# Eurus-Holmes/VAG-NMT

Hardware: AMD Instinct MI355X
Metric: training sentence-pairs/sec (Multi30K en->de, B=64) (higher is better)
Workload: dtype f32; 1 GPU; configs[1]: multimodal en->de train step, B=64/GPU, Ts=Tt=40, E=256, H=512, S=512, I=2048, Vs=8507, V=9391, dropout 0.3/0.5/0.5, tied emb, teacher_force_ratio=1; global_batch=64, parallelism=dp1, hip_graph=True

## Files before the change

### vag-nmt_amd/csrc/api.hip

```cpp
#include "../../include/vag_nmt.h"
#include "api_shared.h"
#include <cstring>

static thread_local VagCallCtx g_base_ctx;
static thread_local VagCallCtx* g_active_ctx = nullptr;
VagCallCtx& vag_ctx() { return g_active_ctx ? *g_active_ctx : g_base_ctx; }
VagCallScope::VagCallScope(VagCallCtx& c) : ctx(c), prev(g_active_ctx) { g_active_ctx = &c; }
VagCallScope::~VagCallScope() {
    (void)vag_loss_defer_flush();
    if (ctx.leaf_on) vag_leaf_drop();
    g_active_ctx = prev;
}
static inline const float* as_f(const vag_half* p) { return reinterpret_cast<const float*>(p); }

VagOptions& vag_opt() {
    static VagOptions o;
    return o;
}

extern "C" {

int vag_version(void) { return 330; }

int vag_set_option(const char* name, int64_t value) {
// ... 45 lines not shown
                   float* d_x, int accumulate_dx, float* g_W, float* g_b, vag_stream_t stream) {
    hipStream_t s = S_(stream);
    VAG_CHECK_ARG(x && W && dy && M >= 0 && N > 0 && K > 0 && (!act || y));
    if (M == 0) return VAG_OK;
    if (act) VAG_TRY(vag_tanh_bwd_launch(y, dy, dy, M * N, nullptr, 0, 0.f, s));
    if (d_x) VAG_TRY(gemm_nn(M, K, N, dy, N, W, K, accumulate_dx ? 1.f : 0.f, d_x, K, s));
    if (g_W) VAG_TRY(gemm_tn_acc(N, K, M, dy, N, x, K, g_W, K, s));
    if (g_b) VAG_TRY(vag_colsum_launch(dy, M, N, N, g_b, s));
    return VAG_OK;
}

int vag_embed_fwd(const int64_t* idx, int64_t n, const float* W, int64_t E, float* out, vag_stream_t stream) {
    return vag_embed_gather_launch(idx, 1, 0, n, 1, W, E, out, nullptr, 0, 0.f, S_(stream));
}
int vag_embed_bwd(const int64_t* idx, int64_t n, const float* d_out, int64_t E, float* g_W, vag_stream_t stream) {
    return vag_embed_scatter_launch(idx, 1, 0, n, 1, d_out, E, g_W, nullptr, 0, 0.f, S_(stream));
}

struct DerivedW {
    float *prep, *wcatT, *whh1T, *encT;
    vag_half *wcat16, *wcatT16, *whh1_16, *whh1T16, *enc16, *encT16;
    int64_t total;
};
static int64_t cgru_prep_total(int64_t H);
static DerivedW derived_layout(float* p, int64_t H) {
    DerivedW w;
    const int64_t C = 2 * H, Q = C + 3 * H;
    WsCarver c(p);
    w.prep = c.take(cgru_prep_total(H)); w.wcatT = c.take(Q * H); w.whh1T = c.take(3 * H * H); w.encT = c.take(2 * 3 * H * H);
    w.wcat16 = c.take_as<vag_half>(Q * H); w.wcatT16 = c.take_as<vag_half>(Q * H);
    w.whh1_16 = c.take_as<vag_half>(3 * H * H); w.whh1T16 = c.take_as<vag_half>(3 * H * H);
    w.enc16 = c.take_as<vag_half>(2 * 3 * H * H); w.encT16 = c.take_as<vag_half>(2 * 3 * H * H);
    w.total = c.off;
    return w;
}

static float* handoff_planes(int64_t need) {
    const VagCallCtx& c = vag_ctx();
    return (need > 0 && c.handoff_planes && c.handoff_floats >= need) ? c.handoff_planes : nullptr;
}

struct BiGruWs {
    float *x, *xp, *hst, *gates, *dgh, *carry, *dx, *whhT, *gx;
    unsigned *sync, *sync_b;
    int64_t total;
};
static BiGruWs bigru_ws(float* ws, int64_t B, int64_t Ts, int64_t E, int64_t H) {
    BiGruWs w;
    WsCarver c(ws);
    w.x = c.take(Ts * B * E);
    w.xp = c.take(Ts * B * 6 * H);
    w.hst = c.take(2 * (Ts + 1) * B * H);
    w.gates = c.take(2 * Ts * 4 * B * H);
    w.dgh = c.take(2 * Ts * B * 3 * H);
    w.carry = c.take(4 * B * H);
    w.dx = c.take(Ts * B * E);
    w.whhT = c.take(2 * 3 * H * H);
    w.gx = c.take(3 * Ts * B * H);
    w.sync = c.take_as<unsigned>(vag_enc_persistent_sync_words(B, Ts));
    w.sync_b = c.take_as<unsigned>(vag_enc_persistent_sync_words(B, Ts));
    w.total = c.off;
    return w;
}
int64_t vag_bigru_ws_floats(int64_t B, int64_t Ts, int64_t E, int64_t H) { return bigru_ws(nullptr, B, Ts, E, H).total; }

int vag_bigru_seq_fwd(const int64_t* src, const int32_t* lengths, const float* emb, vag_gru_w fw, vag_gru_w bw, float p_emb,
                      float p_ctx, const uint64_t* rng, int64_t B, int64_t Ts, int64_t E, int64_t H, float* enc,
                      float* mask, float* ws, vag_stream_t stream) {
    hipStream_t s = S_(stream);
    VAG_CHECK_ARG(src && lengths && emb && enc && mask && ws && B > 0 && Ts > 0 && E > 0 && H > 0);
    VAG_CHECK_ARG(E % 4 == 0 && H % 4 == 0 && aligned16(ws) && aligned16(enc));
    VAG_CHECK_ARG(fw.w_ih && fw.w_hh && fw.b_ih && fw.b_hh && bw.w_ih && bw.w_hh && bw.b_ih && bw.b_hh);
    BiGruWs w = bigru_ws(ws, B, Ts, E, H);
    const int64_t R = Ts * B;
    VAG_TRY(vag_embed_gather_launch(src, 1, Ts, Ts, B, emb, E, w.x, rng, VAG_DROP_ENC_EMB, p_emb, s, mask));
    VagGemmGroup grp0;
    VAG_TRY(vag_gemm_launch(R, 3 * H, E, 1.f, w.x, E, 1, fw.w_ih, 1, E, 0.f, w.xp, 6 * H, fw.b_ih, 0, s));
    VAG_TRY(vag_gemm_launch(R, 3 * H, E, 1.f, w.x, E, 1, bw.w_ih, 1, E, 0.f, w.xp + 3 * H, 6 * H, bw.b_ih, 0, s));
    VAG_TRY(grp0.end(s));
    const int64_t BH = B * H;
    const bool s16 = vag_ctx().store16 && vag_ctx().derived;
    VAG_CHECK_ARG(!vag_ctx().store16 || (vag_ctx().derived && H % 8 == 0));
    if (!s16 && vag_opt().persistent && vag_enc_persistent_ok(B, Ts, H)) {
        return vag_enc_fwd_persistent_launch(w.xp, fw.w_hh, bw.w_hh, fw.b_hh, bw.b_hh, lengths, w.hst, w.gates, enc, w.sync, rng,
                                             p_ctx, B, Ts, H, s);
    }
    const vag_half* w16 = s16 ? derived_layout(const_cast<float*>(vag_ctx().derived), H).enc16 : nullptr;
    if (s16 && vag_opt().persistent && vag_enc_wide16_ok(B, Ts, H) && B >= 64) {
        return vag_enc_fwd_wide16_launch(w.xp, w16, w16 + 3 * H * H, fw.b_hh, bw.b_hh, lengths, w.hst, w.gates, enc,
                                         reinterpret_cast<vag_half*>(w.dgh), w.sync, rng, p_ctx, B, Ts, H, s);
    }
    {
        const VagJob zj[2] = {{nullptr, w.hst, B, H, H, H, 0}, {nullptr, w.hst + (Ts + 1) * BH, B, H, H, H, 0}};
        VAG_TRY(vag_jobs_launch(zj, 2, s));
    }
    GruStepArgs a = {};
    a.lda = H; a.ldw = H; a.ldother = 6 * H; a.ldh = H; a.ld2 = Ts * 2 * H;
    a.M = (int)B; a.K = (int)H; a.H = (int)H; a.lengths = lengths; a.comp_hidden = 1;
    for (int64_t k = 0; k < Ts; ++k) {
        for (int d = 0; d < 2; ++d) {
            const int64_t t = d == 0 ? k : Ts - 1 - k;
            const vag_gru_w& g = d == 0 ? fw : bw;
            float* hs = w.hst + d * (Ts + 1) * BH;
            GruSide& sd = a.s[d];
            sd.A = hs + k * BH; sd.W = s16 ? as_f(w16 + d * 3 * H * H) : g.w_hh; sd.bias = g.b_hh;
            sd.other = w.xp + t * B * 6 * H + d * 3 * H;
            sd.hprev = hs + k * BH; sd.hout = hs + (k + 1) * BH;
            sd.out2 = enc + t * 2 * H + d * H;
            sd.save = w.gates + (d * Ts + k) * 4 * BH;
            sd.t = (int)t;
        }
        VAG_TRY(vag_gru_step_launch(a, 2, s, s16));
    }
    VAG_TRY(vag_dropout_apply_launch(enc, B * Ts * 2 * H, 0, rng, VAG_DROP_ENC_CTX, p_ctx, s));
    return VAG_OK;
}

int vag_bigru_seq_bwd(const int64_t* src, const int32_t* lengths, vag_gru_w fw, vag_gru_w bw, float p_emb, float p_ctx,
                      const uint64_t* rng, int64_t B, int64_t Ts, int64_t E, int64_t H, float* d_enc, float* ws,
                      float* g_emb, vag_gru_g g_fw, vag_gru_g g_bw, vag_stream_t stream) {
    hipStream_t s = S_(stream);
    VAG_CHECK_ARG(src && lengths && d_enc && ws && g_emb && B > 0 && Ts > 0 && E % 4 == 0 && H % 4 == 0);
    BiGruWs w = bigru_ws(ws, B, Ts, E, H);
    const int64_t R = Ts * B, BH = B * H;
    float* d_xp = w.xp;
    const float* whhT = w.whhT;
    const bool s16 = vag_ctx().store16 && vag_ctx().derived;
    VAG_CHECK_ARG(!vag_ctx().store16 || (vag_ctx().derived && H % 8 == 0));
    if (s16) {
        whhT = as_f(derived_layout(const_cast<float*>(vag_ctx().derived), H).encT16);
    } else if (vag_ctx().derived) {
        whhT = derived_layout(const_cast<float*>(vag_ctx().derived), H).encT;
    } else {
        for (int d = 0; d < 2; ++d) {
            const vag_gru_w& g = d == 0 ? fw : bw;
            VAG_TRY(vag_transpose_launch(g.w_hh, 3 * H, H, w.whhT + d * 3 * H * H, s));
        }
    }
    const bool pers_on = vag_opt().persistent && vag_opt().persistent_enc_bwd;
    const bool wide16 = s16 && pers_on && vag_enc_wide16_ok(B, Ts, H) && B >= 64;
    const bool persist = wide16 || (!s16 && pers_on && (H == 512 || H == 256) && vag_enc_persistent_ok(B, Ts, H));
    if (wide16) {
        VAG_TRY(vag_enc_bwd_wide16_launch(reinterpret_cast<const vag_half*>(whhT), d_enc, w.gates, w.hst, lengths, rng, p_ctx, d_xp,
                                          w.dgh, reinterpret_cast<vag_half*>(w.gx), w.sync_b, B, Ts, H, s));
    } else if (persist) {
        VAG_TRY(vag_enc_bwd_persistent_launch(whhT, d_enc, w.gates, w.hst, lengths, rng, p_ctx, d_xp, w.dgh,
                                              handoff_planes(vag_enc_bwd_planes_floats(B, Ts, H)), w.sync_b, B, Ts, H, s));
    }
    GruBwdArgs a = {};
    a.ld_add = Ts * 2 * H; a.ldh = H; a.ldgi = 6 * H; a.ldgh = 3 * H;
    a.M = (int)B; a.H = (int)H; a.lengths = lengths; a.rng = rng; a.sid = VAG_DROP_ENC_CTX; a.p = p_ctx;
    int cur = 0;
    auto cell_of = [&](auto& sd, int d, int64_t k) {
        const int64_t t = d == 0 ? k : Ts - 1 - k;
        sd.dh_add = d_enc + t * 2 * H + d * H;
        sd.drop_idx0 = t * 2 * H + d * H;
        sd.save = w.gates + (d * Ts + k) * 4 * BH;
        sd.hprev = w.hst + (d * (Ts + 1) + k) * BH;
        sd.dgi = d_xp + t * B * 6 * H + d * 3 * H;
        sd.dgh = w.dgh + (d * Ts + k) * B * 3 * H;
        sd.t = (int)t;
    };
    for (int d = 0; d < 2; ++d) {
        GruBwdSide& sd = a.s[d];
        cell_of(sd, d, Ts - 1);
        sd.dh_carry = nullptr;
        sd.dh_prev = w.carry + (d * 2 + cur) * BH;
    }
// ... 381 lines not shown
}

struct CgruBwdScratch {
    float *wcatT, *wpT, *whh1T, *dgi2, *dqgh, *dalpha, *ds, *dgi1, *dgh1, *dh1d, *carry, *de, *dvp, *dwp, *dah, *dencwp, *pbuf;
    float *u_all, *du_all, *duk;
    int64_t total;
};
static CgruBwdScratch cgru_bwd_scratch(float* p, int64_t B, int64_t Ts, int64_t Tt, int64_t E, int64_t H) {
    CgruBwdScratch w;
    const int64_t C = 2 * H, Q = C + 3 * H, R = Tt * B;
    WsCarver c(p);
    w.wcatT = c.take(Q * H); w.wpT = c.take(3 * H * C); w.whh1T = c.take(3 * H * H);
    w.dgi2 = c.take(R * 3 * H); w.dqgh = c.take(R * Q);
    w.dalpha = c.take(B * Ts); w.ds = c.take(R * Ts);
    w.dgi1 = c.take(R * 3 * H); w.dgh1 = c.take(R * 3 * H);
    w.dh1d = c.take(B * H); w.carry = c.take(B * H); w.de = c.take(R * E); w.dvp = c.take(VAG_POST_CHUNKS(Ts) * B * C);
    w.dwp = c.take(3 * H * C);
    w.dah = c.take(R * Ts);
    w.dencwp = c.take(B * Ts * 3 * H);
    w.pbuf = c.take(B * H);
    w.u_all = c.take(R * H); w.du_all = c.take(R * H); w.duk = c.take(B * Ts * H);
    w.total = c.off;
    return w;
}
}
float* vag_cgru_bwd_scratch_de(float* scratch, int64_t B, int64_t Ts, int64_t Tt, int64_t E, int64_t H) {
    return cgru_bwd_scratch(scratch, B, Ts, Tt, E, H).de;
}
float* vag_cgru_bwd_scratch_du(float* scratch, int64_t B, int64_t Ts, int64_t Tt, int64_t E, int64_t H) {
    return cgru_bwd_scratch(scratch, B, Ts, Tt, E, H).du_all;
}
extern "C" {
int64_t vag_cgru_bwd_scratch_floats(int64_t B, int64_t Ts, int64_t Tt, int64_t E, int64_t H) {
    return cgru_bwd_scratch(nullptr, B, Ts, Tt, E, H).total;
}

int vag_cgru_attn_decode_seq_bwd_loop(const float* enc, const float* pe, const float* mask, const float* h0, const int64_t* tok,
                                 vag_dec_w w, int64_t B, int64_t Ts, int64_t Tt, int64_t E, int64_t H, int64_t V,
                                 const float* h2_all, const float* c_all, const float* e_all, float* d_h2_all,
                                 float* d_c_all, const float* d_e_all, float* ws, float* d_enc_out, int accumulate_enc,
                                 float* d_pe, float* d_h0, float* scratch, vag_stream_t stream) {
    hipStream_t s = S_(stream);
    VAG_CHECK_ARG(enc && pe && mask && h0 && tok && h2_all && c_all && e_all && d_h2_all && d_c_all && ws && d_enc_out &&
                  d_pe && d_h0 && scratch && dec_w_ok(w));
    VAG_CHECK_ARG(B > 0 && Ts > 0 && Tt > 0 && E % 4 == 0 && H % 4 == 0 && aligned16(ws) && aligned16(scratch));
    (void)V; (void)mask; (void)d_e_all;
    const int64_t C = 2 * H, Q = C + 3 * H, BH = B * H;
    CgruWs k = cgru_ws(ws, B, Ts, Tt, E, H);
    CgruPrep p = cgru_prep(k.prep, H);
    CgruBwdScratch z = cgru_bwd_scratch(scratch, B, Ts, Tt, E, H);
    const bool s16 = vag_ctx().store16;
    VAG_CHECK_ARG(!s16 || (vag_ctx().derived && H % 8 == 0));
    if (vag_ctx().derived) {
        DerivedW dw = derived_layout(const_cast<float*>(vag_ctx().derived), H);
        p = cgru_prep(dw.prep, H);
        z.wcatT = dw.wcatT; z.whh1T = dw.whh1T;
        if (s16) {
            z.wcatT = const_cast<float*>(as_f(dw.wcatT16)); z.whh1T = const_cast<float*>(as_f(dw.whh1T16));
        }
    } else {
        VAG_TRY(vag_transpose_launch(p.wcat, Q, H, z.wcatT, s));
        VAG_TRY(vag_transpose_launch(w.gru1.w_hh, 3 * H, H, z.whh1T, s));
    }
    const bool persist = !s16 && vag_opt().persistent && vag_opt().persistent_dec_bwd && vag_dec_bwd_persistent_ok(B, Ts, Tt, H);
    if (!persist) {
        GruBwdArgs a = {};
        a.ld_add = H; a.ldh = H; a.ldgi = 3 * H; a.ldgh = Q; a.M = (int)B; a.H = (int)H;
        const int64_t t = Tt - 1;
        GruBwdSide& sd = a.s[0];
        sd.dh_carry = nullptr; sd.dh_add = d_h2_all + t * BH; sd.drop_idx0 = 0;
        sd.save = k.g2 + t * 4 * BH; sd.hprev = k.h1 + t * BH;
        sd.dgi = z.dgi2 + t * B * 3 * H; sd.dgh = z.dqgh + t * B * Q + C; sd.dh_prev = z.dh1d; sd.t = 0;
        VAG_TRY(vag_gru_bwd_elem_launch(a, 1, s));
    }
    GruBwdStepArgs f = {};
    f.ld_add = H; f.ldh = H; f.M = (int)B; f.H = (int)H; f.lengths = nullptr; f.rng = nullptr; f.sid = 0; f.p = 0.f;
    if (C % 4 == 0 && aligned16(enc) && aligned16(d_c_all) && B < 65536)
        VAG_TRY(vag_skinny_batched_launch(B, Tt, Ts, C, d_c_all, B * C, C, enc, C, Ts * C, z.dah, B * Ts, Ts, s));
    else
        VAG_TRY(vag_attn_scores_ex_launch(1, enc, d_c_all, C, nullptr, nullptr, Tt * B, 1, B, Ts, C, nullptr, z.dah, s));
    if (persist) {
        VAG_TRY(vag_dec_bwd_persistent_launch(pe, k.encwp, w.attn_v, z.wcatT, z.whh1T, h0, h2_all, k.h1, k.g1, k.g2, k.qhp, k.alpha,
                                              d_h2_all, z.dah, z.dgi2, z.dqgh, z.ds, z.dgi1, z.dgh1, d_h0, k.dal,
                                              handoff_planes(vag_dec_bwd_planes_floats(B, Tt, H)), k.sync_b, B, Ts, Tt, H, s));
    }
    for (int64_t t = Tt - 1; t >= 0 && !persist; --t) {
        float* dgi2 = z.dgi2 + t * B * 3 * H;
        float* dqgh = z.dqgh + t * B * Q;
        const float* wside = s16 ? as_f(reinterpret_cast<const vag_half*>(z.wcatT) + C) : z.wcatT + C;
        VAG_TRY(vag_attn_dot_side_launch(1, k.encwp, dgi2, 3 * H, nullptr, nullptr, z.dah + t * B * Ts, B, Ts, 3 * H, z.dalpha,
                                         B, H, 3 * H, dqgh + C, Q, wside, Q, nullptr, z.dh1d, z.pbuf, H, s, s16));
        VAG_TRY(vag_attn_dq_launch(pe, k.qhp + t * B * Q, Q, w.attn_v, k.alpha + t * B * Ts, z.dalpha, z.ds + t * B * Ts, B,
                                   Ts, C, dqgh, Q, s, s16));
        f.lda = Q; f.ldw = Q; f.K = (int)C; f.ldgi = 3 * H; f.ldgh = 3 * H; f.has_cell = 1;
        GruBwdStepSide& sd = f.s[0];
        sd.A = dqgh; sd.WT = z.wcatT; sd.addend = z.pbuf; sd.dh_add = nullptr; sd.drop_idx0 = 0;
        sd.save = k.g1 + t * 4 * BH; sd.hprev = (t == 0) ? h0 : h2_all + (t - 1) * BH;
        sd.dgi = z.dgi1 + t * B * 3 * H; sd.dgh = z.dgh1 + t * B * 3 * H; sd.dh_direct = z.carry; sd.dh_out = nullptr; sd.t = 0;
        VAG_TRY(vag_gru_bwd_step_launch(f, 1, s, s16));
        f.lda = 3 * H; f.ldw = 3 * H; f.K = (int)(3 * H);
        sd.A = z.dgh1 + t * B * 3 * H; sd.WT = z.whh1T; sd.addend = z.carry;
        if (t > 0) {
            const int64_t t1 = t - 1;
            f.has_cell = 1; f.ldgi = 3 * H; f.ldgh = Q;
            sd.dh_add = d_h2_all + t1 * BH;
            sd.save = k.g2 + t1 * 4 * BH; sd.hprev = k.h1 + t1 * BH;
            sd.dgi = z.dgi2 + t1 * B * 3 * H; sd.dgh = z.dqgh + t1 * B * Q + C; sd.dh_direct = z.dh1d; sd.dh_out = nullptr;
        } else {
            f.has_cell = 0;
            sd.dh_add = nullptr; sd.save = nullptr; sd.hprev = nullptr; sd.dgi = nullptr; sd.dgh = nullptr;
            sd.dh_direct = nullptr; sd.dh_out = d_h0;
        }
        VAG_TRY(vag_gru_bwd_step_launch(f, 1, s, s16));
    }
    VAG_TRY(vag_attn_post_bwd_launch(pe, k.qhp, Q, w.attn_v, z.ds, k.alpha, d_c_all, B, Ts, Tt, C, d_pe, z.dvp, d_enc_out,
                                     accumulate_enc, s, s16));
    {
        VagGemmGroup now;
        VAG_TRY(gemm_nn(Tt * B, H, 3 * H, z.dgi2, 3 * H, w.gru2.w_ih, H, 0.f, z.du_all, H, s));
        VAG_TRY(now.end(s));
    }
    VAG_TRY(vag_attn_wsum_pair_launch(k.alpha, z.du_all, H, z.duk, k.uk, H, z.u_all, B, Ts, Tt, s));
    vag_ctx().u_all_ready = z.u_all;
    return gemm_nn(B * Ts, C, H, z.duk, H, w.c2h, C, 1.f, d_enc_out, C, s);
}

int vag_cgru_attn_decode_seq_bwd_weights(const float* h0, const int64_t* tok, vag_dec_w w, int64_t B, int64_t Ts, int64_t Tt,
                                         int64_t E, int64_t H, const float* h2_all, const float* c_all, const float* e_all,
                                         const float* d_e_all, float* ws, vag_dec_g g, float* scratch, vag_stream_t stream) {
    hipStream_t s = S_(stream);
    VAG_CHECK_ARG(h0 && tok && h2_all && c_all && e_all && ws && scratch && dec_w_ok(w));
    VAG_CHECK_ARG(g.emb && g.gru1.w_ih && g.gru1.w_hh && g.gru1.b_ih && g.gru1.b_hh && g.attn_h && g.attn_v && g.c2h &&
                  g.gru2.w_ih && g.gru2.w_hh && g.gru2.b_ih && g.gru2.b_hh);
    const int64_t C = 2 * H;
    CgruBwdScratch z = cgru_bwd_scratch(scratch, B, Ts, Tt, E, H);
    VagGemmGroup grp3;
    VAG_TRY(vag_colsum_launch(z.dvp, VAG_POST_CHUNKS(Ts) * B, C, C, g.attn_v, s));
    VAG_TRY(vag_cgru_bwd_weights_chunk(h0, tok, w, B, Ts, Tt, E, H, h2_all, c_all, e_all, d_e_all, ws, g, scratch, 0, Tt, true,
                                       s));
    VAG_TRY(grp3.end(s));
    return vag_cgru_bwd_weights_scatter(tok, B, Ts, Tt, E, H, g, scratch, 0, Tt, s);
}
}

int vag_cgru_bwd_weights_chunk(const float* h0, const int64_t* tok, vag_dec_w w, int64_t B, int64_t Ts, int64_t Tt, int64_t E,
                               int64_t H, const float* h2_all, const float* c_all, const float* e_all, const float* d_e_all,
                               float* ws, vag_dec_g g, float* scratch, int64_t t0, int64_t t1, bool first, hipStream_t s) {
    VAG_CHECK_ARG(0 <= t0 && t0 < t1 && t1 <= Tt);
    const int64_t C = 2 * H, Q = C + 3 * H, r0 = t0 * B, n = (t1 - t0) * B;
    CgruWs k = cgru_ws(ws, B, Ts, Tt, E, H);
    CgruBwdScratch z = cgru_bwd_scratch(scratch, B, Ts, Tt, E, H);
    const float* dqgh = z.dqgh + r0 * Q;
    const float* dgh2 = dqgh + C;
    const float* dgi2 = z.dgi2 + r0 * 3 * H;
    const float* dgi1 = z.dgi1 + r0 * 3 * H;
    const float* dgh1 = z.dgh1 + r0 * 3 * H;
    const float* h1 = k.h1 + r0 * H;
    VAG_TRY(gemm_tn_acc(3 * H, H, n, dgh2, Q, h1, H, g.gru2.w_hh, H, s, g.gru2.b_hh));
    VAG_TRY(gemm_tn_acc(C, H, n, dqgh, Q, h1, H, g.attn_h, H, s));
    if (first) {
        if (vag_ctx().u_all_ready != z.u_all) VAG_TRY(vag_attn_wsum_launch(1, k.alpha, k.uk, B, Ts, Tt, H, z.u_all, s));
        vag_ctx().u_all_ready = nullptr;
    }
    VAG_TRY(gemm_tn_acc(3 * H, H, n, dgi2, 3 * H, z.u_all + r0 * H, H, g.gru2.w_ih, H, s, g.gru2.b_ih));
    VAG_TRY(gemm_tn_acc(H, C, n, z.du_all + r0 * H, H, c_all + r0 * C, C, g.c2h, C, s));
    if (h0 + B * H == h2_all) {
        VAG_TRY(gemm_tn_acc(3 * H, H, n, dgh1, 3 * H, h0 + r0 * H, H, g.gru1.w_hh, H, s, g.gru1.b_hh));
// ... 563 lines not shown
int vag_sample_step_p_dev(const float* const* logp, const int64_t* ldl, int64_t M, int64_t* toks, float* token_logp,
                          int32_t* di_state, int64_t max_len, int64_t* tok_out, int64_t B, int64_t n, int64_t V, float temperature,
                          int64_t top_k, const uint64_t* rng, int32_t* n_alive, float top_p, int32_t* set_size,
                          vag_stream_t stream) {
    VAG_CHECK_ARG(di_state != nullptr);
    return vag_sample_step_p_launch(logp, ldl, M, toks, token_logp, 0, di_state, max_len, nullptr, nullptr, nullptr, tok_out, B, n,
                                    V, temperature, top_k, rng, n_alive, top_p, set_size, S_(stream));
}
int vag_sample_noise(const uint64_t* rng, int64_t di, int64_t N, int64_t V, float* out, vag_stream_t stream) {
    return vag_sample_noise_launch(rng, di, N, V, out, S_(stream));
}

int vag_mbr_supported(int64_t Nh, int64_t Lh, int64_t Nr, int64_t Lr) { return vag_mbr_supported_host(Nh, Lh, Nr, Lr); }
int vag_mbr_select(const int64_t* hyps, const int64_t* refs, const float* weights, int64_t B, int64_t Nh, int64_t Lh, int64_t Nr,
                   int64_t Lr, int utility, int32_t* matches, float* util, float* expected, int64_t* best, vag_stream_t stream) {
    return vag_mbr_select_launch(hyps, refs, weights, B, Nh, Lh, Nr, Lr, utility, matches, util, expected, best, S_(stream));
}

int vag_corpus_bleu_supported(int64_t Lh, int64_t R, int64_t Lr) { return vag_corpus_bleu_supported_host(Lh, R, Lr); }
int vag_corpus_bleu_stats(const int64_t* hyps, const int64_t* refs, const int32_t* n_refs, int64_t N, int64_t Lh, int64_t R,
                          int64_t Lr, int32_t* per_sentence, int64_t* totals, vag_stream_t stream) {
    return vag_corpus_bleu_stats_launch(hyps, refs, n_refs, N, Lh, R, Lr, per_sentence, totals, S_(stream));
}

int vag_surface_expand(const int64_t* rows, int64_t R, int64_t L, const int32_t* off, const int32_t* chars, int64_t V, int32_t* out,
                       int64_t C, int32_t* lens, vag_stream_t stream) {
    return vag_surface_expand_launch(rows, R, L, off, chars, V, out, C, lens, S_(stream));
}
int vag_chrf_supported(int64_t Nh, int64_t Ch, int64_t Nr, int64_t Cr) { return vag_chrf_supported_host(Nh, Ch, Nr, Cr); }
int vag_chrf_max_chars(void) { return vag_chrf_max_chars_host(); }
int vag_chrf_select(const int32_t* hchars, const int32_t* hlens, const int32_t* rchars, const int32_t* rlens, const float* weights,
                    int64_t B, int64_t Nh, int64_t Ch, int64_t Nr, int64_t Cr, int32_t* matches, float* util, float* expected,
                    int64_t* best, vag_stream_t stream) {
    return vag_chrf_select_launch(hchars, hlens, rchars, rlens, weights, B, Nh, Ch, Nr, Cr, matches, util, expected, best, S_(stream));
}

int vag_mrt_weights(const float* nll, const float* cost, const float* valid, int64_t B, int64_t Tt, int64_t N, float alpha, float scale,
                    float* inv_cnt, float* q, float* risk, vag_stream_t stream) {
    VAG_CHECK_ARG(risk != nullptr);
    return vag_mrt_weights_launch(nll, cost, valid, B, Tt, N, alpha, scale, inv_cnt, q, risk, nullptr, 0.f, 0, S_(stream));
}
int vag_mrt_pack(const int64_t* cand, int64_t G, int64_t Nc, int64_t L, const int64_t* gold, int64_t Tg, int include_gold, int64_t* tgt,
                 int64_t Tt, float* valid, vag_stream_t stream) {
    return vag_mrt_pack_launch(cand, G, Nc, L, gold, Tg, include_gold, tgt, Tt, valid, S_(stream));
}

int vag_clip_adam_flat(float* p, float* g, float* m, float* v, int64_t n, int nseg, const int64_t* seg_off,
                       const float* seg_lr, const float* seg_wd, float clip, float grad_scale, float beta1, float beta2,
                       float eps, int zero_grad, int32_t* step, float* norm_out, void* scratch, const float* lr_dev,
                       vag_stream_t stream) {
    return vag_clip_adam_launch(p, g, m, v, n, nseg, seg_off, seg_lr, seg_wd, clip, grad_scale, beta1, beta2, eps, zero_grad,
                                step, norm_out, scratch, lr_dev, S_(stream));
}

int vag_clip_adam_flat_ema(float* p, float* g, float* m, float* v, int64_t n, int nseg, const int64_t* seg_off,
                           const float* seg_lr, const float* seg_wd, float clip, float grad_scale, float beta1, float beta2,
                           float eps, int zero_grad, int32_t* step, float* norm_out, void* scratch, const float* lr_dev,
                           float* ema, float ema_decay, int ema_warmup, vag_stream_t stream) {
    return vag_clip_adam_ema_launch(p, g, m, v, n, nseg, seg_off, seg_lr, seg_wd, clip, grad_scale, beta1, beta2, eps, zero_grad,
                                    step, norm_out, scratch, lr_dev, ema, ema_decay, ema_warmup, S_(stream));
}

int vag_swap_flat(float* a, float* b, int64_t n, vag_stream_t stream) { return vag_swap_flat_launch(a, b, n, S_(stream)); }

int vag_clip_adam_shard(float* p, float* g, float* m, float* v, int64_t n, int nseg, const int64_t* seg_off, const float* seg_lr,
                        const float* seg_wd, float clip, float grad_scale, float beta1, float beta2, float eps, int zero_grad,
                        int32_t* step, float* norm_out, void* scratch, const float* lr_dev, int64_t lo, int64_t hi, int phase,
                        double* sumsq, vag_stream_t stream) {
    return vag_clip_adam_shard_launch(p, g, m, v, n, nseg, seg_off, seg_lr, seg_wd, clip, grad_scale, beta1, beta2, eps, zero_grad,
                                      step, norm_out, scratch, lr_dev, lo, hi, phase, sumsq, S_(stream));
}

int vag_copy4(const void* const* src, void* const* dst, const int64_t* bytes, int n, vag_stream_t stream) {
    return vag_copy4_launch(src, dst, bytes, n, S_(stream));
}

int vag_recurrence_supported(int kind, int64_t B, int64_t Ts, int64_t Tt, int64_t H) {
    if (kind == 0) return vag_enc_persistent_ok(B, Ts, H) ? 1 : 0;
    if (kind == 1) return vag_dec_persistent_ok(B, Ts, Tt, H) ? 1 : 0;
    return 0;
}
int vag_persistent_timeouts(void) { return vag_persistent_timeouts_read(); }
int64_t vag_handoff_planes_floats(int64_t B, int64_t Ts, int64_t Tt, int64_t H) {
    const int64_t e = vag_enc_bwd_planes_floats(B, Ts, H), d = vag_dec_bwd_planes_floats(B, Tt, H);
    return e > d ? e : d;
}
int vag_set_handoff_planes(float* buf, int64_t floats) {
    VAG_CHECK_ARG((buf == nullptr || (floats > 0 && aligned16(buf))));
    g_base_ctx.handoff_planes = buf;
    g_base_ctx.handoff_floats = buf ? floats : 0;
    return VAG_OK;
}
int vag_set_operator_guard(void* guard) {
    VAG_CHECK_ARG((reinterpret_cast<uintptr_t>(guard) & 3) == 0);
    g_base_ctx.guard = reinterpret_cast<unsigned*>(guard);
    return VAG_OK;
}
int vag_gemm_group_plan(int n, const int64_t* M, const int64_t* N, const int64_t* K, const int* accumulate, int* split,
                        int* order) {
    return vag_gemm_group_plan_host(n, M, N, K, accumulate, split, order);
}
int vag_gemm_plan(int64_t M, int64_t N, int64_t K, int a_kc, int b_kc, int vec, float beta, int act, int c_half, int a_bf16,
                  int rowsum, int planes, int* plan) {
    return vag_gemm_plan_host(M, N, K, a_kc, b_kc, vec, beta, act, c_half, a_bf16, rowsum, planes, plan);
}
int vag_recurrence_time(int kind, double* ms_total, int* launches) { return vag_persistent_time_read(kind, ms_total, launches); }
int64_t vag_recurrence_sync_words(int kind, int64_t B, int64_t T) {
    return kind == 0 ? vag_enc_persistent_sync_words(B, T) : vag_dec_persistent_sync_words(B, T);
}
int vag_cgru_recurrence_fwd(const float* pe, const float* mask, const float* h0, const float* xp1, vag_dec_w w, const float* wcat,
                            const float* bcat, const float* encwp, int64_t B, int64_t Ts, int64_t Tt, int64_t H, float* h1,
                            float* g1, float* qhp, float* alpha, float* h2_all, float* g2, float* psc, void* sync,
                            vag_stream_t stream) {
    VAG_CHECK_ARG(dec_w_ok(w) && vag_dec_persistent_ok(B, Ts, Tt, H));
    return vag_dec_fwd_persistent_launch(pe, mask, h0, xp1, w.gru1.w_hh, w.gru1.b_hh, wcat, bcat, w.attn_v, encwp, w.gru2.b_ih, h1,
                                         g1, qhp, alpha, h2_all, g2, psc, reinterpret_cast<unsigned*>(sync), B, Ts, Tt, H,
                                         S_(stream));
}

int vag_dropout_mask(const uint64_t* rng, int which, int64_t n, float p, float* out, vag_stream_t stream) {
    VAG_CHECK_ARG(which >= 1 && which <= 3);
    return vag_dropout_mask_launch(rng, which, n, p, out, S_(stream));
}
int vag_rng_advance(uint64_t* rng, vag_stream_t stream) { return vag_rng_advance_launch(rng, S_(stream)); }

}
```

### vag-nmt_amd/csrc/common.h

```cpp
#pragma once
#include <hip/hip_runtime.h>
#include <stdint.h>
#include <stddef.h>

#define VAG_OK 0
#define VAG_EINVAL (-22)
#define VAG_ENOSYS (-38)

#define VAG_CHECK_ARG(cond)                     \
    do {                                        \
        if (!(cond)) return VAG_EINVAL;         \
    } while (0)

#define VAG_LAUNCH_CHECK()                                  \
    do {                                                    \
        hipError_t e__ = hipGetLastError();                 \
        if (e__ != hipSuccess) return (int)e__;             \
    } while (0)

#define VAG_TRY(expr)                  \
    do {                               \
        int r__ = (expr);              \
        if (r__ != 0) return r__;      \
    } while (0)

typedef float f32x4 __attribute__((ext_vector_type(4)));
typedef float f32x16 __attribute__((ext_vector_type(16)));

static inline int64_t cdiv64(int64_t a, int64_t b) { return (a + b - 1) / b; }
static inline bool aligned16(const void* p) { return (((uintptr_t)p) & 15) == 0; }

template <bool MAX>
__device__ __forceinline__ float wave_allreduce(float v) {
#define VAG_DPP_ROR(N) __builtin_bit_cast(float, __builtin_amdgcn_update_dpp(0, __builtin_bit_cast(int, v), 0x120 + (N), 0xf, 0xf, false))
    { const float o = VAG_DPP_ROR(8); v = MAX ? fmaxf(v, o) : v + o; }
    { const float o = VAG_DPP_ROR(4); v = MAX ? fmaxf(v, o) : v + o; }
    { const float o = VAG_DPP_ROR(2); v = MAX ? fmaxf(v, o) : v + o; }
    { const float o = VAG_DPP_ROR(1); v = MAX ? fmaxf(v, o) : v + o; }
#undef VAG_DPP_ROR
    float a = v, b = v;
    asm volatile("s_nop 1\n\tv_permlane16_swap_b32 %0, %1\n\ts_nop 1" : "+v"(a), "+v"(b));
    v = MAX ? fmaxf(a, b) : a + b;
    a = v; b = v;
    asm volatile("s_nop 1\n\tv_permlane32_swap_b32 %0, %1\n\ts_nop 1" : "+v"(a), "+v"(b));
    return MAX ? fmaxf(a, b) : a + b;
}
__device__ __forceinline__ float quad_sum(float v) {
    v += __builtin_bit_cast(float, __builtin_amdgcn_update_dpp(0, __builtin_bit_cast(int, v), 0xB1, 0xf, 0xf, false));
    v += __builtin_bit_cast(float, __builtin_amdgcn_update_dpp(0, __builtin_bit_cast(int, v), 0x4E, 0xf, 0xf, false));
    return v;
}
__device__ __forceinline__ float wave_sum(float v) { return wave_allreduce<false>(v); }
__device__ __forceinline__ float wave_max(float v) { return wave_allreduce<true>(v); }
__device__ __forceinline__ float vag_tanh(float x) {
    float e = __expf(2.0f * x);
    return 1.0f - 2.0f * __builtin_amdgcn_rcpf(e + 1.0f);
}
__device__ __forceinline__ float vag_sigmoid(float x) { return __builtin_amdgcn_rcpf(1.0f + __expf(-x)); }

__device__ __host__ __forceinline__ uint64_t vag_mix64(uint64_t z) {
    z += 0x9E3779B97F4A7C15ull;
    z = (z ^ (z >> 30)) * 0xBF58476D1CE4E5B9ull;
    z = (z ^ (z >> 27)) * 0x94D049BB133111EBull;
    return z ^ (z >> 31);
}
__device__ __forceinline__ float vag_drop_mul(const uint64_t* rng, uint32_t stream_id, uint64_t idx, float p) {
    if (rng == nullptr || p <= 0.0f) return 1.0f;
    uint64_t key = vag_mix64(rng[0] ^ (rng[1] * 0xD1342543DE82EF95ull) ^ ((uint64_t)stream_id << 56));
    uint64_t r = vag_mix64(key + idx);
    float u = (float)(r >> 40) * (1.0f / 16777216.0f);
    return (u >= p) ? 1.0f / (1.0f - p) : 0.0f;
}

typedef _Float16 vag_half;
__device__ __forceinline__ float h16_lo(unsigned p) { return (float)__builtin_bit_cast(vag_half, (unsigned short)(p & 0xffffu)); }
__device__ __forceinline__ float h16_hi(unsigned p) { return (float)__builtin_bit_cast(vag_half, (unsigned short)(p >> 16)); }
template <bool XH> __device__ __forceinline__ float4 ld4_any(const float* base, int64_t elem) {
    if (XH) {
        const uint2 p = *reinterpret_cast<const uint2*>(reinterpret_cast<const vag_half*>(base) + elem);
        return make_float4(h16_lo(p.x), h16_hi(p.x), h16_lo(p.y), h16_hi(p.y));
    }
    return *reinterpret_cast<const float4*>(base + elem);
}
template <bool XH> __device__ __forceinline__ float ld1_any(const float* base, int64_t elem) {
    if (XH) return (float)reinterpret_cast<const vag_half*>(base)[elem];
    return base[elem];
}

struct VagOptions {
    int gemm_f32mfma = 0;
    int gemm_big = 1;
    int gemm_slabs = 1;
    int gemm_nogroup = 0;
    int gemm_force_tile = 0;
    int gemm_force_splitk = 0;
    int gemm_debug = 0;
    int64_t head_chunk = -1;
    int head_fuse = 1;
    int head_bf16_grads = 1;
    int persistent = 1;
    int persistent_dec_bwd = 1;
    int persistent_enc_bwd = 1;
    int attn_dot_reg = 1;
    int handoff_planes = 1;
    int free_persistent = 1;
    int s16_one_plane = 1;
    int head_bf16_dlogits = 1;
    int leaf_queue = 1;
    int attn_row = 1;
    int loss_ride = 1;
    int dec_xcd_map = 33;
    int step_fork = 0;
    int64_t persist_spin_limit = 0;
    int persist_timing = 0;
    int64_t dec_bwd_stamps = 0;
    int64_t dec_stamps = 0;
};
VagOptions& vag_opt();

enum { VAG_ACT_NONE = 0, VAG_ACT_TANH = 1 };
enum { VAG_DROP_ENC_EMB = 1, VAG_DROP_ENC_CTX = 2, VAG_DROP_DEC_OUT = 3 };

int vag_gemm_launch(int64_t M, int64_t N, int64_t K, float alpha, const float* A, int64_t sam, int64_t sak,
                    const float* B, int64_t sbk, int64_t sbn, float beta, float* C, int64_t ldc,
                    const float* bias, int act, hipStream_t stream, int c_half = 0,
                    float* rowsum = nullptr,
                    int a_bf16 = 0);
int vag_gemm_launch_planes(int planes, int64_t M, int64_t N, int64_t K, float alpha, const float* A, int64_t sam, int64_t sak,
                           const float* B, int64_t sbk, int64_t sbn, float beta, float* C, int64_t ldc, hipStream_t stream,
                           int a_bf16 = 0);
int64_t vag_logits_parts_count(int64_t M, int64_t N, int64_t K, const float* A, int64_t lda, const float* W, int64_t ldw);
int vag_logits_parts_launch(int64_t M, int64_t N, int64_t K, const float* A, int64_t lda, const float* W, int64_t ldw,
                            const float* bias, float* out, int64_t ldo, float* parts, hipStream_t stream);
int vag_skinny_launch(int64_t M, int64_t N, int64_t K, const float* A, int64_t lda, const float* W, int64_t ldw,
                      const float* bias, const float* addend, int64_t ldadd, float* out, int64_t ldo, int act,
                      hipStream_t stream, bool w16 = false);
int vag_attn_dot_side_launch(int mode, const float* x, const float* q, int64_t ldq, const float* v, const float* mask,
                             const float* addend, int64_t N, int64_t Ts, int64_t W, float* out, int64_t M, int64_t Np,
                             int64_t K, const float* A, int64_t lda, const float* Wt, int64_t ldw, const float* pbias,
                             const float* padd, float* P, int64_t ldp, hipStream_t stream, bool s16 = false);
int vag_skinny_gather_launch(int64_t M, int64_t N, int64_t K, const float* table, int64_t ldt, const int64_t* idx, const float* W,
                             int64_t ldw, const float* bias, float* out, int64_t ldo, float* gathered, int64_t ldg,
                             hipStream_t stream);
int vag_skinny3_launch(int64_t M, int64_t N, const float* const* A, const int64_t* lda, const float* const* W, const int64_t* ldw,
                       const int64_t* K, const float* const* bias, float* out, int64_t ldo, int act, const uint64_t* rng, int sid,
                       float p, int64_t drop_idx0, hipStream_t stream, const float* addend = nullptr, int64_t ldadd = 0,
                       const float* addend2 = nullptr, const int64_t* idx2 = nullptr, int64_t ldadd2 = 0);
int vag_skinny_batched_launch(int64_t nb, int64_t M, int64_t N, int64_t K, const float* A, int64_t lda, int64_t bsA,
                              const float* W, int64_t ldw, int64_t bsW, float* out, int64_t ldo, int64_t bsO,
                              hipStream_t stream);
int vag_skinny_nn_launch(int64_t M, int64_t N, int64_t K, const float* A, int64_t lda, const float* B, int64_t ldb,
                         float beta, float* C, int64_t ldc, hipStream_t stream,
                         float* out2 = nullptr, int64_t ldo2 = 0, float scale2 = 0.f, int acc2 = 0);
void vag_gemm_group_begin();
int vag_gemm_group_end(hipStream_t stream);
void vag_gemm_group_abort();
struct VagGemmGroup {
    bool open = true;
    explicit VagGemmGroup(bool enable = true) : open(enable) { if (enable) vag_gemm_group_begin(); }
    int end(hipStream_t s) { if (!open) return VAG_OK; open = false; return vag_gemm_group_end(s); }
    ~VagGemmGroup() { if (open) vag_gemm_group_abort(); }
    VagGemmGroup(const VagGemmGroup&) = delete;
    VagGemmGroup& operator=(const VagGemmGroup&) = delete;
};
int vag_leaf_flush(hipStream_t stream);
void vag_leaf_drop();
int vag_colsum_launch(const float* X, int64_t M, int64_t N, int64_t ld, float* out, hipStream_t stream);
int vag_colsum3_launch(const float* X, int64_t M, int64_t N, int64_t ld, float* out, float* out2, float* out3,
                       hipStream_t stream);
int vag_transpose_launch(const float* in, int64_t M, int64_t N, float* out, hipStream_t stream);

struct GruSide {
    const float* A;
    const float* W;
    const float* bias;
    const float* other;
    const int64_t* other_idx;
    const float* hprev;
    float* hout;
    float* out2;
    float* save;
    int t;
};
struct GruStepArgs {
    GruSide s[2];
    int64_t lda, ldw, ldother, ldh, ld2;
    int M, K, H;
// ... 29 lines not shown
```

### vag-nmt_amd/csrc/kernels.h

```cpp
#pragma once
#include "common.h"
#include "call_ctx.h"
#include "../../include/vag_nmt.h"

static inline int64_t round64(int64_t n) { return (n + 63) & ~63ll; }
struct WsCarver {
    float* base;
    int64_t off = 0;
    explicit WsCarver(float* b) : base(b) {}
    float* take(int64_t n) {
        float* q = base ? base + off : nullptr;
        off += round64(n);
        return q;
    }
    template <class T> T* take_as(int64_t n) {
        return reinterpret_cast<T*>(take((n * (int64_t)sizeof(T) + 3) / 4));
    }
};
struct DecTables {
    float *embp, *embw3, *encw2;
    unsigned long long* cand;
    int64_t total;
};
DecTables vag_dec_tables(float* base, int64_t B, int64_t Ts, int64_t Tt, int64_t E, int64_t H, int64_t V, bool token_only = false);
// ... 63 lines not shown
                           int64_t N, int64_t rps, int64_t Ts, int64_t C, float* scores, hipStream_t s);
int vag_attn_scores_ex_launch(int mode, const float* pe, const float* q, int64_t ldq, const float* v, const float* mask,
                              int64_t N, int64_t rps, int64_t rows_mod, int64_t Ts, int64_t C, const float* addend,
                              float* scores, hipStream_t s);
int vag_attn_ctx_gru_launch(const float* scores, const float* encwp, int64_t N, int64_t rps, int64_t Ts, int64_t H,
                            const float* b_ih, const float* hp, int64_t ldhp, const float* hprev, float* alpha, float* hout,
                            float* save, hipStream_t s, bool x16 = false,
                            const float* x2 = nullptr, int64_t W2 = 0, float* out2 = nullptr);
int vag_attn_wsum_launch(int over_src, const float* a, const float* x, int64_t B, int64_t Ts, int64_t T, int64_t W, float* out,
                         hipStream_t s);
int vag_attn_ctx_launch(int softmax, const float* scores, const float* enc, int64_t N, int64_t rps, int64_t Ts,
                        int64_t C, float* alpha, float* ctx, hipStream_t s);
int vag_softmax_bwd_launch(const float* alpha, const float* dalpha, int64_t N, int64_t Ts, float* dscore, hipStream_t s);
int vag_attn_dq_launch(const float* pe, const float* q, int64_t ldq, const float* v, const float* alpha,
                       const float* dalpha, float* dscore, int64_t N, int64_t Ts, int64_t C, float* dq, int64_t lddq,
                       hipStream_t s, bool x16 = false);
int vag_attn_post_bwd_launch(const float* pe, const float* q_all, int64_t ldq, const float* v, const float* ds_all,
                             const float* alpha_all, const float* dc_all, int64_t B, int64_t Ts, int64_t Tt,
                             int64_t C, float* d_pe, float* dvp, float* d_enc, int accumulate_enc, hipStream_t s,
                             bool x16 = false);
int vag_outer2_launch(const float* a1, const float* x1, const float* a2, const float* x2, int64_t B, int64_t Ts,
                      int64_t C, float* out, int accumulate, hipStream_t s);

inline bool vag_label_smoothing_ok(float eps) { return eps >= 0.f && eps < 1.f; }
int vag_lse_nll_launch(const float* logits, int64_t ldl, int64_t rows, int64_t V, const int64_t* tgt, int64_t B,
                       int64_t Tt, const float* vw, float* lse, float* nll, int64_t* argmax, int64_t argmax_stride,
                       float* logp_out, int64_t ldlp, hipStream_t s, float eps);
int vag_inv_cnt_launch(const int64_t* tgt, int64_t B, int64_t Tt, float* inv_cnt, hipStream_t s);
int vag_loss_mt_launch(const LossTask& t, float* loss, hipStream_t s);
int vag_ce_bwd_launch(float* logits, int64_t ldl, int64_t rows, int64_t V, const int64_t* tgt, int64_t B, int64_t Tt,
                      const float* vw, const float* lse, const float* inv_cnt, const float* d_loss, hipStream_t s,
                      float eps);
int vag_ce_bwd_colsum_launch(float* logits, int64_t ldl, int64_t rows, int64_t V, const int64_t* tgt, int64_t B, int64_t Tt,
                             const float* vw, const float* lse, const float* inv_cnt, const float* d_loss, float* g_bias,
                             hipStream_t s, void* out16, float eps);

int vag_logsoftmax_bwd_launch(const float* logp, int64_t ldlp, float* d, int64_t ldd, int64_t rows, int64_t V,
                              hipStream_t s);

inline bool vag_kd_ok(int64_t K, float lambda, int64_t V) { return K >= 1 && K <= 64 && K <= V && lambda > 0.f && lambda <= 1.f; }
int vag_kd_nll_launch(const float* logits, int64_t ldl, int64_t rows, int64_t V, const int64_t* tgt, int64_t B, int64_t Tt,
                      const float* vw, const float* lse, const int32_t* idx, const float* q, int64_t K, float lambda, float* nll,
                      hipStream_t s);
int vag_kd_dlogits_launch(float* dlogits, int64_t ldl, int64_t rows, int64_t V, const int64_t* tgt, int64_t B, int64_t Tt,
                          const float* vw, const float* inv_cnt, const float* d_loss, const int32_t* idx, const float* q, int64_t K,
                          float lambda, float* g_bias, hipStream_t s);

int vag_token_conf_launch(const float* const* logits, const int64_t* ldl, const float* const* lse, int64_t M, const int64_t* tgt,
                          int64_t B, int64_t Tt, int64_t V, float* token_logp, float* entropy, int32_t* rank, int32_t* top,
                          float* top_logp, float* sent, hipStream_t s);

inline bool vag_rdrop_ok(float alpha) { return alpha > 0.f && alpha < INFINITY; }
int vag_rdrop_pair_launch(const float* logits, int64_t ldl, int64_t rows, int64_t V, const int64_t* tgt, int64_t B, int64_t Tt,
                          const float* vw, const float* lse, float alpha, float* kl, float* nll, hipStream_t s);
int vag_rdrop_bwd_colsum_launch(float* logits, int64_t ldl, int64_t rows, int64_t V, const int64_t* tgt, int64_t B, int64_t Tt,
                                const float* vw, const float* lse, const float* kl, const float* inv_cnt, const float* d_loss,
                                float alpha, float* g_bias, hipStream_t s, float eps);

int vag_l2norm_fwd_launch(const float* y, int64_t B, int64_t S, float* nrm, float* out, hipStream_t s);
int vag_l2norm_bwd_launch(const float* y, const float* nrm, const float* out, const float* d_out, int64_t B, int64_t S,
                          int act, float* dy, hipStream_t s);
int vag_rank_loss_launch(const float* scores, int64_t B, float margin, int kind, float* G, float* loss, hipStream_t s,
                         const float* g_scale = nullptr, float scale = 1.f);
int vag_retrieval_rank_launch(const float* scores, int64_t N, int* ranks, hipStream_t s);
int vag_scale_by_dev_launch(float* x, int64_t n, const float* scalar, hipStream_t s);

int vag_clip_adam_shard_launch(float* p, float* g, float* m, float* v, int64_t n, int nseg, const int64_t* seg_off,
                               const float* seg_lr, const float* seg_wd, float clip, float grad_scale, float beta1, float beta2,
                               float eps, int zero_grad, int32_t* step, float* norm_out, void* scratch, const float* lr_dev,
                               int64_t lo, int64_t hi, int phase, double* sumsq, hipStream_t s);
int vag_clip_adam_launch(float* p, float* g, float* m, float* v, int64_t n, int nseg, const int64_t* seg_off,
                         const float* seg_lr, const float* seg_wd, float clip, float grad_scale, float beta1,
                         float beta2, float eps, int zero_grad, int32_t* step, float* norm_out, void* scratch, const float* lr_dev,
                         hipStream_t s);
int vag_clip_adam_ema_launch(float* p, float* g, float* m, float* v, int64_t n, int nseg, const int64_t* seg_off,
                             const float* seg_lr, const float* seg_wd, float clip, float grad_scale, float beta1,
                             float beta2, float eps, int zero_grad, int32_t* step, float* norm_out, void* scratch,
                             const float* lr_dev, float* ema, float ema_decay, int ema_warmup, hipStream_t s);
int vag_swap_flat_launch(float* a, float* b, int64_t n, hipStream_t s);

bool vag_enc_persistent_ok(int64_t B, int64_t Ts, int64_t H);
int64_t vag_enc_persistent_sync_words(int64_t B, int64_t Ts);
int vag_enc_fwd_persistent_launch(const float* xp, const float* w_fw, const float* w_bw, const float* b_fw, const float* b_bw,
                                  const int* lengths, float* hst, float* gates, float* enc, unsigned* sync, const uint64_t* rng,
                                  float p_ctx, int64_t B, int64_t Ts, int64_t H, hipStream_t s);
int vag_enc_bwd_persistent_launch(const float* whhT, const float* d_enc, const float* gates, const float* hst, const int* lengths,
                                  const uint64_t* rng, float p_ctx, float* d_xp, float* dgh, float* planes, unsigned* sync, int64_t B,
                                  int64_t Ts, int64_t H, hipStream_t s);
int64_t vag_enc_bwd_planes_floats(int64_t B, int64_t Ts, int64_t H);
int64_t vag_dec_bwd_planes_floats(int64_t B, int64_t Tt, int64_t H);
bool vag_enc_wide16_ok(int64_t B, int64_t Ts, int64_t H);
int vag_enc_fwd_wide16_launch(const float* xp, const vag_half* w16_fw, const vag_half* w16_bw, const float* b_fw, const float* b_bw,
                              const int* lengths, float* hst, float* gates, float* enc, vag_half* hx, unsigned* sync, const uint64_t* rng,
                              float p_ctx, int64_t B, int64_t Ts, int64_t H, hipStream_t s);
int vag_enc_bwd_wide16_launch(const vag_half* wt16, const float* d_enc, const float* gates, const float* hst, const int* lengths,
                              const uint64_t* rng, float p_ctx, float* d_xp, float* dgh, vag_half* gx, unsigned* sync, int64_t B,
                              int64_t Ts, int64_t H, hipStream_t s);
int vag_gemm_group_plan_host(int n, const int64_t* M, const int64_t* N, const int64_t* K, const int* accumulate, int* split,
                             int* order);
int vag_gemm_plan_host(int64_t M, int64_t N, int64_t K, int a_kc, int b_kc, int vec, float beta, int act, int c_half, int a_bf16,
                       int rowsum, int planes, int* plan);
int vag_persistent_timeouts_read(void);
unsigned* vag_persist_guard(void);
int vag_persistent_time_read(int kind, double* ms_total, int* launches);
bool vag_dec_bwd_persistent_ok(int64_t B, int64_t Ts, int64_t Tt, int64_t H);
int vag_dec_bwd_persistent_launch(const float* pe, const float* encwp, const float* v, const float* wcatT, const float* whh1T,
                                  const float* h0, const float* h2_all, const float* h1, const float* g1, const float* g2,
                                  const float* qhp, const float* alpha, const float* d_h2_all, const float* dah, float* dgi2,
                                  float* dqgh, float* ds, float* dgi1, float* dgh1, float* d_h0, float* dal, float* planes,
                                  unsigned* sync, int64_t B, int64_t Ts, int64_t Tt, int64_t H, hipStream_t s);
float* vag_cgru_bwd_scratch_de(float* scratch, int64_t B, int64_t Ts, int64_t Tt, int64_t E, int64_t H);
float* vag_cgru_bwd_scratch_du(float* scratch, int64_t B, int64_t Ts, int64_t Tt, int64_t E, int64_t H);
int vag_attn_dot_row_launch(bool bwd, const float* x, const float* q, int64_t ldq, const float* mask, const float* alpha, int64_t B,
                            int64_t Ts, int64_t C, float* wout, float* sum, hipStream_t s);
int vag_rank_bwd_launch(const float* G, const float* im, const float* sv, const float* d_loss, int64_t B, int64_t S, float* d_im,
                        float* d_s, hipStream_t s);
int vag_attn_wsum_pair_launch(const float* a, const float* y, int64_t Wy, float* out_src, const float* x, int64_t Wx, float* out_time,
                              int64_t B, int64_t Ts, int64_t T, hipStream_t s);
int vag_loss_defer_flush();
bool vag_attn_row_gru_ok(int64_t N, int64_t Ts, int64_t H, int64_t W2);
int vag_attn_row_gru_launch(const float* pe, const float* q, int64_t ldq, const float* v, const float* mask, const float* keys,
                            const float* x2, int64_t N, int64_t rps, int64_t Ts, int64_t H, int64_t W2, const float* b_ih,
                            const float* hp, int64_t ldhp, const float* hprev, float* alpha, float* hout, float* out2, hipStream_t s);
int vag_rmw_defer_flush(hipStream_t s);
bool vag_rmw_defer_meanpool(const float* mask, const float* dx, float coef, int64_t B, int64_t Ts, int64_t C, float* out, int accumulate);
void vag_step_zero_ranges(float* ws_enc, float* ws_dec, int64_t B, int64_t Ts, int64_t Tt, int64_t Es, int64_t Et, int64_t H,
                          unsigned** p, int64_t* n);
bool vag_dec_persistent_ok(int64_t B, int64_t Ts, int64_t Tt, int64_t H);
int64_t vag_dec_persistent_sync_words(int64_t B, int64_t Tt);
int vag_dec_fwd_persistent_launch(const float* pe, const float* mask, const float* h0, const float* xp1, const float* W1,
                                  const float* b1, const float* wcat, const float* bcat, const float* v, const float* encwp,
                                  const float* b_ih2, float* h1, float* g1, float* qhp, float* alpha, float* h2_all, float* g2,
                                  float* psc, unsigned* sync, int64_t B, int64_t Ts, int64_t Tt, int64_t H, hipStream_t s);
bool vag_dec_free_persistent_ok(int64_t B, int64_t Ts, int64_t Tt, int64_t E, int64_t H, int64_t V);
int vag_dec_free_persistent_launch(const float* pe, const float* mask, const float* h0, const float* W1, const float* b1,
                                   const float* wcat, const float* bcat, const float* v, const float* encwp, const float* b_ih2,
                                   float* h1, float* g1, float* qhp, float* alpha, float* h2_all, float* g2, float* psc,
                                   unsigned* sync, const DecTables& tab, const float* hw1, const float* hb1, const float* hb2,
                                   const float* hb3, const float* out_w, const float* out_b, float* tmid, float* logits, int64_t ldl,
                                   int64_t* tok, const uint64_t* rng, float p_out, int64_t B, int64_t Ts, int64_t Tt, int64_t E,
                                   int64_t H, int64_t V, hipStream_t s);

int64_t vag_beam_scratch_bytes_impl(int64_t B, int64_t k, int64_t V);
int vag_beam_step_launch(float* logp, int64_t ldl, float* nll, int64_t* beam, int64_t di, int32_t* di_state,
                         int64_t max_len, const float* h_in, float* h_out, int64_t* tok_out, int64_t B, int64_t k,
                         int64_t V, int64_t H, int32_t* n_alive, void* scratch, hipStream_t s, const float* parts = nullptr,
                         int64_t nparts = 0, int flags = 0);
int vag_beam_finish_launch(const float* nll, const int64_t* beam, int64_t max_len, int64_t steps, int64_t B, int64_t k,
                           int64_t* out, float* best, hipStream_t s);
int vag_beam_ens_step_launch(const float* const* logp, const int64_t* ldl, int64_t M, float* nll, int64_t* beam, int64_t di,
                             int32_t* di_state, int64_t max_len, const float* const* h_in, float* const* h_out, const int64_t* H,
                             int64_t* tok_out, int64_t B, int64_t k, int64_t V, int32_t* n_alive, void* scratch, hipStream_t s,
                             int flags = 0);
int vag_beam_finish_nbest_launch(const float* nll, const int64_t* beam, int64_t max_len, int64_t steps, int64_t B, int64_t k,
                                 int64_t n, int64_t* out, float* scores, hipStream_t s);
int vag_beam_finish_nbest_slots_launch(const float* nll, const int64_t* beam, int64_t max_len, int64_t steps, int64_t B, int64_t k,
                                       int64_t n, int64_t* out, float* scores, int64_t* slots, hipStream_t s);
int64_t vag_beam_div_scratch_bytes_impl(int64_t B, int64_t k, int64_t V);
int vag_beam_div_step_launch(const float* const* logp, const int64_t* ldl, int64_t M, float* nll, int64_t* beam, int64_t di,
                             int32_t* di_state, int64_t max_len, const float* const* h_in, float* const* h_out, const int64_t* H,
                             int64_t* tok_out, int64_t B, int64_t k, int64_t V, int32_t* n_alive, void* scratch, int flags,
                             int64_t groups, float strength, hipStream_t s);
int64_t vag_beam_req_scratch_bytes_impl(int64_t B, int64_t k, int64_t V);
int vag_beam_req_step_launch(const float* const* logp, const int64_t* ldl, int64_t M, float* nll, int64_t* beam, int64_t di,
                             int32_t* di_state, int64_t max_len, const float* const* h_in, float* const* h_out, const int64_t* H,
                             int64_t* tok_out, int64_t B, int64_t k, int64_t V, int32_t* n_alive, void* scratch, int flags,
                             const int64_t* required, int32_t* state, hipStream_t s);
int64_t vag_beam_sbs_scratch_bytes_impl(int64_t B, int64_t k, int64_t V);
int vag_beam_sbs_step_launch(const float* const* logp, const int64_t* ldl, int64_t M, float* nll, int64_t* beam, int64_t di,
                             int32_t* di_state, int64_t max_len, const float* const* h_in, float* const* h_out, const int64_t* H,
                             int64_t* tok_out, int64_t B, int64_t k, int64_t V, int32_t* n_alive, void* scratch, int flags,
                             const uint64_t* rng, float* gum, hipStream_t s);
int64_t vag_beam_pen_scratch_bytes_impl(int64_t B, int64_t k, int64_t V);
int vag_beam_cover_launch(const float* const* alpha, int64_t M, const float* mask, const float* cov, const int64_t* beam, int64_t di,
                          const int32_t* di_state, int64_t max_len, int64_t B, int64_t k, int64_t Tp, float beta, float* cov_row,
                          float* cp_row, hipStream_t s);
int vag_beam_pen_step_launch(const float* const* logp, const int64_t* ldl, int64_t M, float* nll, int64_t* beam, int64_t di,
                             int32_t* di_state, int64_t max_len, const float* const* h_in, float* const* h_out, const int64_t* H,
                             int64_t* tok_out, int64_t B, int64_t k, int64_t V, int32_t* n_alive, void* scratch, int flags,
                             int32_t* lens, const float* cp_row, float* cpen, const float* cov_row, float* cov, int64_t Tp,
                             const float* lp, const float* bonus, int stepwise, hipStream_t s);
int vag_beam_finish_pen_launch(const float* nll, const int64_t* beam, const int32_t* lens, const float* cpen, const float* lp,
                               const float* bonus, int64_t max_len, int64_t steps, int64_t B, int64_t k, int64_t n, int64_t* out,
                               float* scores, int64_t* slots, float* logp, int32_t* length, float* cp, hipStream_t s);
int vag_beam_constrain_launch(float* const* logp, const int64_t* ldl, int64_t M, const int64_t* beam, int64_t di,
                              const int32_t* di_state, bool dev_form, int64_t max_len, int64_t B, int64_t k, int64_t V,
                              const int64_t* prefix, int64_t Lp, const int64_t* phrases, const int32_t* phrase_sent, int64_t P,
                              int64_t ngram, hipStream_t s);
int vag_forced_score_launch(const float* const* logits, const int64_t* ldl, const float* const* lse, int64_t M,
                            const int64_t* tgt, int64_t B, int64_t Tt, int64_t V, float* token_logp, float* logp, float* score,
                            hipStream_t s);
int vag_beam_attn_record_launch(const float* const* alpha, int64_t M, float* attn_hist, int64_t di, const int32_t* di_state,
                                int64_t max_len, int64_t B, int64_t k, int64_t Tp, hipStream_t s);
// ... 84 lines not shown
```

### vag-nmt_amd/csrc/persist.hip

```cpp
#include "kernels.h"
#include "gemm_shared.h"
#include <algorithm>
#include <atomic>
#include <mutex>

namespace {

typedef unsigned __attribute__((address_space(1))) gu32;
#define RLX_AGENT __ATOMIC_RELAXED, __HIP_MEMORY_SCOPE_AGENT

constexpr unsigned SPIN_LIMIT = 1u << 19;
__device__ unsigned g_persist_timeouts;
__device__ unsigned g_persist_guard[2];
__device__ __forceinline__ void note_timeout(unsigned* err, unsigned* guard) {
    __hip_atomic_store((gu32*)err, 1u, RLX_AGENT);
    __hip_atomic_store((gu32*)guard, 1u, RLX_AGENT);
    atomicAdd(guard + 1, 1u);
    atomicAdd(&g_persist_timeouts, 1u);
}

struct EncPArgs {
    const float* xp;
    const float* W[2];
    const float* bias[2];
    const int* lengths;
    float* hst;
    float* gates;
    float* enc;
    unsigned* cnt;
    unsigned* err;
    unsigned* guard;
    unsigned spin;
    const uint64_t* rng;
    float p_ctx;
    int B, Ts, H, RT, CS;
    int rt0, RTP;
};

template <int N> __device__ __forceinline__ void ld_rows_sc1(const float* p, float4 (&a)[N], float4 (&b)[N]);
template <> __device__ __forceinline__ void ld_rows_sc1<1>(const float* p, float4 (&a)[1], float4 (&b)[1]) {
    asm volatile("global_load_dwordx4 %0, %2, off sc1\n\tglobal_load_dwordx4 %1, %2, off offset:16 sc1\n\ts_waitcnt vmcnt(0)"
                 : "=&v"(a[0]), "=&v"(b[0]) : "v"(p) : "memory");
}
template <> __device__ __forceinline__ void ld_rows_sc1<2>(const float* p, float4 (&a)[2], float4 (&b)[2]) {
    asm volatile("global_load_dwordx4 %0, %4, off sc1\n\tglobal_load_dwordx4 %1, %4, off offset:16 sc1\n\t"
                 "global_load_dwordx4 %2, %4, off offset:128 sc1\n\tglobal_load_dwordx4 %3, %4, off offset:144 sc1\n\t"
                 "s_waitcnt vmcnt(0)"
                 : "=&v"(a[0]), "=&v"(b[0]), "=&v"(a[1]), "=&v"(b[1]) : "v"(p) : "memory");
}
template <> __device__ __forceinline__ void ld_rows_sc1<3>(const float* p, float4 (&a)[3], float4 (&b)[3]) {
    asm volatile("global_load_dwordx4 %0, %6, off sc1\n\tglobal_load_dwordx4 %1, %6, off offset:16 sc1\n\t"
                 "global_load_dwordx4 %2, %6, off offset:128 sc1\n\tglobal_load_dwordx4 %3, %6, off offset:144 sc1\n\t"
                 "global_load_dwordx4 %4, %6, off offset:256 sc1\n\tglobal_load_dwordx4 %5, %6, off offset:272 sc1\n\t"
                 "s_waitcnt vmcnt(0)"
                 : "=&v"(a[0]), "=&v"(b[0]), "=&v"(a[1]), "=&v"(b[1]), "=&v"(a[2]), "=&v"(b[2]) : "v"(p) : "memory");
}
template <> __device__ __forceinline__ void ld_rows_sc1<4>(const float* p, float4 (&a)[4], float4 (&b)[4]) {
    asm volatile("global_load_dwordx4 %0, %8, off sc1\n\tglobal_load_dwordx4 %1, %8, off offset:16 sc1\n\t"
                 "global_load_dwordx4 %2, %8, off offset:128 sc1\n\tglobal_load_dwordx4 %3, %8, off offset:144 sc1\n\t"
                 "global_load_dwordx4 %4, %8, off offset:256 sc1\n\tglobal_load_dwordx4 %5, %8, off offset:272 sc1\n\t"
                 "global_load_dwordx4 %6, %8, off offset:384 sc1\n\tglobal_load_dwordx4 %7, %8, off offset:400 sc1\n\t"
                 "s_waitcnt vmcnt(0)"
                 : "=&v"(a[0]), "=&v"(b[0]), "=&v"(a[1]), "=&v"(b[1]), "=&v"(a[2]), "=&v"(b[2]), "=&v"(a[3]), "=&v"(b[3])
                 : "v"(p) : "memory");
}
template <> __device__ __forceinline__ void ld_rows_sc1<6>(const float* p, float4 (&a)[6], float4 (&b)[6]) {
    asm volatile("global_load_dwordx4 %0, %12, off sc1\n\tglobal_load_dwordx4 %1, %12, off offset:16 sc1\n\t"
                 "global_load_dwordx4 %2, %12, off offset:128 sc1\n\tglobal_load_dwordx4 %3, %12, off offset:144 sc1\n\t"
                 "global_load_dwordx4 %4, %12, off offset:256 sc1\n\tglobal_load_dwordx4 %5, %12, off offset:272 sc1\n\t"
                 "global_load_dwordx4 %6, %12, off offset:384 sc1\n\tglobal_load_dwordx4 %7, %12, off offset:400 sc1\n\t"
                 "global_load_dwordx4 %8, %12, off offset:512 sc1\n\tglobal_load_dwordx4 %9, %12, off offset:528 sc1\n\t"
                 "global_load_dwordx4 %10, %12, off offset:640 sc1\n\tglobal_load_dwordx4 %11, %12, off offset:656 sc1\n\t"
                 "s_waitcnt vmcnt(0)"
                 : "=&v"(a[0]), "=&v"(b[0]), "=&v"(a[1]), "=&v"(b[1]), "=&v"(a[2]), "=&v"(b[2]), "=&v"(a[3]), "=&v"(b[3]),
                   "=&v"(a[4]), "=&v"(b[4]), "=&v"(a[5]), "=&v"(b[5])
                 : "v"(p) : "memory");
}
template <int N>
__device__ __forceinline__ void ld_rows_tagged(const float* p, float4 (&a)[N], float4 (&b)[N], unsigned spin, bool& dead,
                                               unsigned* err, unsigned* guard);
__device__ __forceinline__ void st_sc1(__amdgpu_buffer_rsrc_t r, unsigned byte_off, float4 v) {
    const u32x4 u = {__builtin_bit_cast(unsigned, v.x), __builtin_bit_cast(unsigned, v.y), __builtin_bit_cast(unsigned, v.z),
                     __builtin_bit_cast(unsigned, v.w)};
    __builtin_amdgcn_raw_buffer_store_b128(u, r, byte_off, 0, 16);
}
__device__ __forceinline__ void st_sc1_f4(float* p, float4 v) {
    const f32x4 x = {v.x, v.y, v.z, v.w};
    asm volatile("global_store_dwordx4 %0, %1, off sc1\n\ts_nop 1" :: "v"(p), "v"(x) : "memory");
}
#ifndef VAG_TAGGED
#define VAG_TAGGED 1
#endif
__device__ __forceinline__ float tag1(float x) { return VAG_TAGGED ? __uint_as_float(__float_as_uint(x) | 1u) : x; }
__device__ __forceinline__ float4 tag4(float4 v) { return make_float4(tag1(v.x), tag1(v.y), tag1(v.z), tag1(v.w)); }
__device__ __forceinline__ unsigned tagbits(float4 v) {
    return __float_as_uint(v.x) & __float_as_uint(v.y) & __float_as_uint(v.z) & __float_as_uint(v.w);
}
template <int N>
__device__ __forceinline__ void ld_rows_tagged(const float* p, float4 (&a)[N], float4 (&b)[N], unsigned spin, bool& dead,
                                               unsigned* err, unsigned* guard) {
    for (unsigned tries = 0;; ++tries) {
        ld_rows_sc1<N>(p, a, b);
        if (!VAG_TAGGED) return;
        unsigned m = 1u;
#pragma unroll
        for (int s = 0; s < N; ++s) m &= tagbits(a[s]) & tagbits(b[s]);
        if (__all((m & 1u) != 0u) || dead) return;
        if (tries > spin) { if ((threadIdx.x & 63) == 0) note_timeout(err, guard); dead = true; return; }
    }
}
__device__ __forceinline__ void st_sc1_f1(float* p, float v) {
    asm volatile("global_store_dword %0, %1, off sc1\n\ts_nop 1" :: "v"(p), "v"(v) : "memory");
}
__device__ __forceinline__ int ld_row(int lane) { return 4 * ((lane >> 2) & 3) + (lane >> 4); }
__device__ __forceinline__ int ld_src4(int lane) { return 4 * (16 * (lane & 3) + 4 * ((lane & 15) >> 2) + (lane >> 4)); }
__device__ __forceinline__ float4 perm4(float4 v, int src4) {
    float4 o;
    o.x = __int_as_float(__builtin_amdgcn_ds_bpermute(src4, __float_as_int(v.x)));
    o.y = __int_as_float(__builtin_amdgcn_ds_bpermute(src4, __float_as_int(v.y)));
    o.z = __int_as_float(__builtin_amdgcn_ds_bpermute(src4, __float_as_int(v.z)));
    o.w = __int_as_float(__builtin_amdgcn_ds_bpermute(src4, __float_as_int(v.w)));
    return o;
}
__device__ __forceinline__ void split8(const float4 a, const float4 b, bf16x8 (&p)[3]) {
    unsigned q[3][4];
    split3(a.x, a.y, q[0][0], q[1][0], q[2][0]);
    split3(a.z, a.w, q[0][1], q[1][1], q[2][1]);
    split3(b.x, b.y, q[0][2], q[1][2], q[2][2]);
    split3(b.z, b.w, q[0][3], q[1][3], q[2][3]);
#pragma unroll
    for (int i = 0; i < 3; ++i) {
        const u32x4 t = {q[i][0], q[i][1], q[i][2], q[i][3]};
        p[i] = __builtin_bit_cast(bf16x8, t);
    }
}
__device__ __forceinline__ f32x4 mma6(const bf16x8 (&a)[3], const bf16x8 (&b)[3], f32x4 acc) {
    acc = __builtin_amdgcn_mfma_f32_16x16x32_bf16(a[0], b[2], acc, 0, 0, 0);
    acc = __builtin_amdgcn_mfma_f32_16x16x32_bf16(a[1], b[1], acc, 0, 0, 0);
    acc = __builtin_amdgcn_mfma_f32_16x16x32_bf16(a[2], b[0], acc, 0, 0, 0);
    acc = __builtin_amdgcn_mfma_f32_16x16x32_bf16(a[0], b[1], acc, 0, 0, 0);
    acc = __builtin_amdgcn_mfma_f32_16x16x32_bf16(a[1], b[0], acc, 0, 0, 0);
    acc = __builtin_amdgcn_mfma_f32_16x16x32_bf16(a[0], b[0], acc, 0, 0, 0);
    return acc;
}

constexpr int PL_PLANE_BYTES = 64 * 16, PL_KSTEP_BYTES = 3 * PL_PLANE_BYTES;
__host__ __device__ constexpr int64_t pl_block_bytes(int64_t K) { return (K / 32) * PL_KSTEP_BYTES; }
typedef unsigned u32x2 __attribute__((ext_vector_type(2)));
__device__ __forceinline__ unsigned pl_slot_off(int r, int k0) { return (unsigned)((r + 16 * ((k0 & 31) >> 3)) * 16 + 8 * ((k0 >> 2) & 1)); }
__device__ __forceinline__ void st_planes4(const char* kblk, unsigned voff, float4 v) {
    unsigned q[3][2];
    split3(v.x, v.y, q[0][0], q[1][0], q[2][0]);
    split3(v.z, v.w, q[0][1], q[1][1], q[2][1]);
    const u32x2 x0 = {q[0][0], q[0][1]}, x1 = {q[1][0], q[1][1]}, x2 = {q[2][0], q[2][1]};
    asm volatile("global_store_dwordx2 %0, %1, %4 sc1\n\tglobal_store_dwordx2 %0, %2, %4 offset:1024 sc1\n\t"
                 "global_store_dwordx2 %0, %3, %4 offset:2048 sc1\n\ts_nop 1"
                 :: "v"(voff), "v"(x0), "v"(x1), "v"(x2), "s"(kblk) : "memory");
}
#define VAG_PLD(o, v, a, off) "global_load_dwordx4 %" #o ", %" #v ", %" #a " offset:" #off " sc1\n\t"
template <int N> __device__ __forceinline__ void ld_planes_sc1(const char* p, unsigned voff, u32x4 (&f)[3 * N]);
template <> __device__ __forceinline__ void ld_planes_sc1<2>(const char* p, unsigned voff, u32x4 (&f)[6]) {
    const char* p1 = p + 8192;
    asm volatile(VAG_PLD(0, 6, 7, 0) VAG_PLD(1, 6, 7, 1024) VAG_PLD(2, 6, 7, 2048) VAG_PLD(3, 6, 7, 3072) VAG_PLD(4, 6, 8, -4096) VAG_PLD(5, 6, 8, -3072)
                 "s_waitcnt vmcnt(0)"
                 : "=&v"(f[0]), "=&v"(f[1]), "=&v"(f[2]), "=&v"(f[3]), "=&v"(f[4]), "=&v"(f[5]) : "v"(voff), "s"(p), "s"(p1) : "memory");
}
template <> __device__ __forceinline__ void ld_planes_sc1<3>(const char* p, unsigned voff, u32x4 (&f)[9]) {
    const char* p1 = p + 8192;
    asm volatile(VAG_PLD(0, 9, 10, 0) VAG_PLD(1, 9, 10, 1024) VAG_PLD(2, 9, 10, 2048) VAG_PLD(3, 9, 10, 3072) VAG_PLD(4, 9, 11, -4096)
                 VAG_PLD(5, 9, 11, -3072) VAG_PLD(6, 9, 11, -2048) VAG_PLD(7, 9, 11, -1024) VAG_PLD(8, 9, 11, 0)
                 "s_waitcnt vmcnt(0)"
                 : "=&v"(f[0]), "=&v"(f[1]), "=&v"(f[2]), "=&v"(f[3]), "=&v"(f[4]), "=&v"(f[5]), "=&v"(f[6]), "=&v"(f[7]), "=&v"(f[8])
                 : "v"(voff), "s"(p), "s"(p1) : "memory");
}
template <> __device__ __forceinline__ void ld_planes_sc1<4>(const char* p, unsigned voff, u32x4 (&f)[12]) {
    const char* p1 = p + 8192;
    asm volatile(VAG_PLD(0, 12, 13, 0) VAG_PLD(1, 12, 13, 1024) VAG_PLD(2, 12, 13, 2048) VAG_PLD(3, 12, 13, 3072) VAG_PLD(4, 12, 14, -4096)
                 VAG_PLD(5, 12, 14, -3072) VAG_PLD(6, 12, 14, -2048) VAG_PLD(7, 12, 14, -1024) VAG_PLD(8, 12, 14, 0) VAG_PLD(9, 12, 14, 1024)
                 VAG_PLD(10, 12, 14, 2048) VAG_PLD(11, 12, 14, 3072)
                 "s_waitcnt vmcnt(0)"
                 : "=&v"(f[0]), "=&v"(f[1]), "=&v"(f[2]), "=&v"(f[3]), "=&v"(f[4]), "=&v"(f[5]), "=&v"(f[6]), "=&v"(f[7]), "=&v"(f[8]),
                   "=&v"(f[9]), "=&v"(f[10]), "=&v"(f[11])
                 : "v"(voff), "s"(p), "s"(p1) : "memory");
}
template <> __device__ __forceinline__ void ld_planes_sc1<6>(const char* p, unsigned voff, u32x4 (&f)[18]) {
    const char *p1 = p + 8192, *p2 = p + 16384;
    asm volatile(VAG_PLD(0, 18, 19, 0) VAG_PLD(1, 18, 19, 1024) VAG_PLD(2, 18, 19, 2048) VAG_PLD(3, 18, 19, 3072) VAG_PLD(4, 18, 20, -4096)
                 VAG_PLD(5, 18, 20, -3072) VAG_PLD(6, 18, 20, -2048) VAG_PLD(7, 18, 20, -1024) VAG_PLD(8, 18, 20, 0) VAG_PLD(9, 18, 20, 1024)
                 VAG_PLD(10, 18, 20, 2048) VAG_PLD(11, 18, 20, 3072) VAG_PLD(12, 18, 21, -4096) VAG_PLD(13, 18, 21, -3072)
                 VAG_PLD(14, 18, 21, -2048) VAG_PLD(15, 18, 21, -1024) VAG_PLD(16, 18, 21, 0) VAG_PLD(17, 18, 21, 1024)
                 "s_waitcnt vmcnt(0)"
                 : "=&v"(f[0]), "=&v"(f[1]), "=&v"(f[2]), "=&v"(f[3]), "=&v"(f[4]), "=&v"(f[5]), "=&v"(f[6]), "=&v"(f[7]), "=&v"(f[8]),
                   "=&v"(f[9]), "=&v"(f[10]), "=&v"(f[11]), "=&v"(f[12]), "=&v"(f[13]), "=&v"(f[14]), "=&v"(f[15]), "=&v"(f[16]), "=&v"(f[17])
                 : "v"(voff), "s"(p), "s"(p1), "s"(p2) : "memory");
}
#undef VAG_PLD
template <int N>
__device__ __forceinline__ f32x4 mma6_planes(const bf16x8 (&w)[N][3], const u32x4 (&f)[3 * N], f32x4 acc) {
#pragma unroll
    for (int s = 0; s < N; ++s) {
        const bf16x8 hf[3] = {__builtin_bit_cast(bf16x8, f[3 * s]), __builtin_bit_cast(bf16x8, f[3 * s + 1]),
                              __builtin_bit_cast(bf16x8, f[3 * s + 2])};
        acc = mma6(w[s], hf, acc);
    }
    return acc;
}

template <int KS>
__global__ __launch_bounds__(512, 1) void enc_fwd_persistent_kernel(EncPArgs a) {
    __shared__ __attribute__((aligned(16))) float lds[21504];
    const int wg = blockIdx.x;
    const int cs = wg % a.CS, rt = a.rt0 + (wg / a.CS) % a.RTP, d = wg / (a.CS * a.RTP);
    const int lane = threadIdx.x & 63, wave = threadIdx.x >> 6;
    const int H = a.H, B = a.B, Ts = a.Ts;
    const int m0 = rt * 16, u0 = cs * 16;
    const int fr = lane & 15, fg = lane >> 4;
    const int kbase = wave * (H >> 3);
    const int64_t BH = (int64_t)B * H;

    bf16x8 wf[KS][3][3];
    {
        const float* W = a.W[d];
#pragma unroll
        for (int s = 0; s < KS; ++s)
#pragma unroll
            for (int j = 0; j < 3; ++j) {
                const float* p = W + (int64_t)(j * H + u0 + fr) * H + kbase + 32 * s + 8 * fg;
                split8(*reinterpret_cast<const float4*>(p), *reinterpret_cast<const float4*>(p + 4), wf[s][j]);
            }
    }
    const int erow = lane >> 2, equad = lane & 3, eslot = erow + 16 * equad;
    const int em = m0 + erow, eu = u0 + 4 * equad;
    const bool eok = wave == 0 && em < B;
    float4 bb[3] = {make_float4(0, 0, 0, 0), make_float4(0, 0, 0, 0), make_float4(0, 0, 0, 0)};
    int len = 0;
    if (eok) {
#pragma unroll
        for (int j = 0; j < 3; ++j) bb[j] = *reinterpret_cast<const float4*>(a.bias[d] + j * H + eu);
        len = a.lengths[em];
    }
    float4 hp = make_float4(0.f, 0.f, 0.f, 0.f);

    float* hs = a.hst + (int64_t)d * (Ts + 1) * BH;
    if (eok) *reinterpret_cast<float4*>(hs + (int64_t)em * H + eu) = hp;
    const __amdgpu_buffer_rsrc_t rs = __builtin_amdgcn_make_buffer_rsrc(hs, 0, (unsigned)((int64_t)(Ts + 1) * BH * 4), 0x00020000);
    gu32* cnt = (gu32*)(a.cnt + ((int64_t)d * a.RT + rt) * Ts);
    const int lrow = min(m0 + ld_row(lane), B - 1);
    const int src4 = ld_src4(lane);
    float4* red = reinterpret_cast<float4*>(lds);
    bool dead = false;

    for (int k = 0; k < Ts; ++k) {
        const int t = d == 0 ? k : Ts - 1 - k;
        float4 xo[3];
        if (eok) {
            const float* xp = a.xp + ((int64_t)t * B + em) * 6 * H + d * 3 * H + eu;
#pragma unroll
            for (int j = 0; j < 3; ++j) xo[j] = *reinterpret_cast<const float4*>(xp + j * H);
        }
        if (k > 0) {
            if (threadIdx.x == 0 && !dead) {
                unsigned spins = 0;
                while (__hip_atomic_load(cnt + (k - 1), RLX_AGENT) < (unsigned)a.CS) {
                    if (++spins > a.spin) { note_timeout(a.err, a.guard); dead = true; break; }
                }
            }
            __syncthreads();
        }
        f32x4 acc[3] = {{0.f, 0.f, 0.f, 0.f}, {0.f, 0.f, 0.f, 0.f}, {0.f, 0.f, 0.f, 0.f}};
        float4 h0[KS], h1[KS];
        if (k > 0) {
            ld_rows_sc1<KS>(hs + ((int64_t)k * B + lrow) * H + kbase + 8 * (lane & 3), h0, h1);
        } else {
#pragma unroll
            for (int s = 0; s < KS; ++s) h0[s] = h1[s] = make_float4(0.f, 0.f, 0.f, 0.f);
        }
#pragma unroll
        for (int s = 0; s < KS; ++s) {
            bf16x8 hf[3];
            split8(perm4(h0[s], src4), perm4(h1[s], src4), hf);
#pragma unroll
            for (int j = 0; j < 3; ++j) acc[j] = mma6(wf[s][j], hf, acc[j]);
        }
#pragma unroll
        for (int j = 0; j < 3; ++j) red[(wave * 3 + j) * 64 + lane] = make_float4(acc[j][0], acc[j][1], acc[j][2], acc[j][3]);
        __syncthreads();
        if (wave == 0) {
            float4 c[3];
#pragma unroll
            for (int j = 0; j < 3; ++j) {
                float4 sum = red[j * 64 + eslot];
#pragma unroll
                for (int w = 1; w < 8; ++w) {
                    const float4 o = red[(w * 3 + j) * 64 + eslot];
                    sum.x += o.x; sum.y += o.y; sum.z += o.z; sum.w += o.w;
                }
                c[j] = make_float4(sum.x + bb[j].x, sum.y + bb[j].y, sum.z + bb[j].z, sum.w + bb[j].w);
            }
            if (eok) {
                const bool active = t < len;
                const float cr[4] = {c[0].x, c[0].y, c[0].z, c[0].w}, cz[4] = {c[1].x, c[1].y, c[1].z, c[1].w};
                const float cn[4] = {c[2].x, c[2].y, c[2].z, c[2].w};
                const float xr[4] = {xo[0].x, xo[0].y, xo[0].z, xo[0].w}, xz[4] = {xo[1].x, xo[1].y, xo[1].z, xo[1].w};
                const float xn[4] = {xo[2].x, xo[2].y, xo[2].z, xo[2].w};
                const float hpv[4] = {hp.x, hp.y, hp.z, hp.w};
                float rr[4], zz[4], nn[4], ho[4], o2[4];
#pragma unroll
                for (int i = 0; i < 4; ++i) {
                    rr[i] = vag_sigmoid(cr[i] + xr[i]);
                    zz[i] = vag_sigmoid(cz[i] + xz[i]);
                    nn[i] = vag_tanh(xn[i] + rr[i] * cn[i]);
                    const float hn = (1.f - zz[i]) * nn[i] + zz[i] * hpv[i];
                    ho[i] = active ? hn : hpv[i];
                    o2[i] = active ? hn : 0.f;
                }
                hp = make_float4(ho[0], ho[1], ho[2], ho[3]);
                const int64_t o = (int64_t)em * H + eu;
                st_sc1(rs, (unsigned)((((int64_t)(k + 1) * B) * H + o) * 4), hp);
                asm volatile("s_waitcnt vmcnt(0)" ::: "memory");
                if (lane == 0) __hip_atomic_fetch_add(cnt + k, 1u, RLX_AGENT);
                float* sv = a.gates + ((int64_t)(d * Ts + k) * 4) * BH + o;
                *reinterpret_cast<float4*>(sv) = make_float4(rr[0], rr[1], rr[2], rr[3]);
                *reinterpret_cast<float4*>(sv + BH) = make_float4(zz[0], zz[1], zz[2], zz[3]);
                *reinterpret_cast<float4*>(sv + 2 * BH) = make_float4(nn[0], nn[1], nn[2], nn[3]);
                *reinterpret_cast<float4*>(sv + 3 * BH) = c[2];
                const int64_t eo = ((int64_t)em * Ts + t) * 2 * H + d * H + eu;
                if (a.rng && a.p_ctx > 0.f) {
#pragma unroll
                    for (int i = 0; i < 4; ++i) o2[i] *= vag_drop_mul(a.rng, VAG_DROP_ENC_CTX, (uint64_t)eo + i, a.p_ctx);
                }
                *reinterpret_cast<float4*>(a.enc + eo) = make_float4(o2[0], o2[1], o2[2], o2[3]);
            }
        }
    }
}

struct EncWArgs {
    const float* xp;
    const vag_half* W16[2];
    const float* bias[2];
    const int* lengths;
    float* hst;
    float* gates;
    float* enc;
    vag_half* hx;
    unsigned* cnt;
    unsigned* err;
    unsigned* guard;
    unsigned spin;
    int B, Ts, H, RG, CS;
    const uint64_t* rng;
    float p_ctx;
};
typedef _Float16 h16x8 __attribute__((ext_vector_type(8)));
template <int N> __device__ __forceinline__ void ld16_sc1(const vag_half* p, u32x4 (&v)[N]);
template <> __device__ __forceinline__ void ld16_sc1<4>(const vag_half* p, u32x4 (&v)[4]) {
    asm volatile("global_load_dwordx4 %0, %4, off sc1\n\tglobal_load_dwordx4 %1, %4, off offset:64 sc1\n\t"
                 "global_load_dwordx4 %2, %4, off offset:128 sc1\n\tglobal_load_dwordx4 %3, %4, off offset:192 sc1\n\t"
                 "s_waitcnt vmcnt(0)"
                 : "=&v"(v[0]), "=&v"(v[1]), "=&v"(v[2]), "=&v"(v[3]) : "v"(p) : "memory");
}
template <> __device__ __forceinline__ void ld16_sc1<8>(const vag_half* p, u32x4 (&v)[8]) {
    asm volatile("global_load_dwordx4 %0, %8, off sc1\n\tglobal_load_dwordx4 %1, %8, off offset:64 sc1\n\t"
                 "global_load_dwordx4 %2, %8, off offset:128 sc1\n\tglobal_load_dwordx4 %3, %8, off offset:192 sc1\n\t"
                 "global_load_dwordx4 %4, %8, off offset:256 sc1\n\tglobal_load_dwordx4 %5, %8, off offset:320 sc1\n\t"
                 "global_load_dwordx4 %6, %8, off offset:384 sc1\n\tglobal_load_dwordx4 %7, %8, off offset:448 sc1\n\t"
                 "s_waitcnt vmcnt(0)"
                 : "=&v"(v[0]), "=&v"(v[1]), "=&v"(v[2]), "=&v"(v[3]), "=&v"(v[4]), "=&v"(v[5]), "=&v"(v[6]), "=&v"(v[7])
                 : "v"(p) : "memory");
}
__device__ __forceinline__ void st_sc1_h4(vag_half* p, float a, float b, float c, float d) {
    typedef unsigned u32x2 __attribute__((ext_vector_type(2)));
    const u32x2 v = {pack_f16(a, b), pack_f16(c, d)};
    asm volatile("global_store_dwordx2 %0, %1, off sc1\n\ts_nop 1" :: "v"(p), "v"(v) : "memory");
}

template <int KST>
__global__ __launch_bounds__(512, 1) void enc_fwd_wide16_kernel(EncWArgs a) {
    extern __shared__ __attribute__((aligned(16))) float wide_lds[];
    const int wg = blockIdx.x;
    const int cs = wg % a.CS, rg = (wg / a.CS) % a.RG, d = wg / (a.CS * a.RG);
    const int lane = threadIdx.x & 63, wave = threadIdx.x >> 6;
    const int kq = wave & 3, ch = wave >> 2;
    const int er = wave & 3, ech = wave >> 2;
    const int H = a.H, B = a.B, Ts = a.Ts;
    const int fr = lane & 15, fg = lane >> 4;
    const int u0 = cs * 32, m0 = rg * 64;
    const int kbase = kq * (H >> 2);
    const int64_t BH = (int64_t)B * H;

    h16x8 wf[KST][3];
    {
        const vag_half* W = a.W16[d];
#pragma unroll
        for (int s = 0; s < KST; ++s)
#pragma unroll
            for (int j = 0; j < 3; ++j) {
                const uint4 q = *reinterpret_cast<const uint4*>(W + (int64_t)(j * H + u0 + 16 * ch + fr) * H + kbase + 32 * s + 8 * fg);
                const u32x4 t = {q.x, q.y, q.z, q.w};
                wf[s][j] = __builtin_bit_cast(h16x8, t);
            }
    }
    const int em = m0 + 16 * er + fr, eu = u0 + 16 * ech + 4 * fg;
// ... 1006 lines not shown
            const int r = tx / 24, col = tx - r * 24;
            const float* al = sc_s + r * Ts;
            const float* ew = ew_s + (int64_t)r * Ts * 24 + col;
            float s0 = 0.f, s1 = 0.f;
            int sp = 0;
            for (; sp + 1 < Ts; sp += 2) { s0 += al[sp] * ew[sp * 24]; s1 += al[sp + 1] * ew[(sp + 1) * 24]; }
            if (sp < Ts) s0 += al[sp] * ew[sp * 24];
            gi_s[tx] = s0 + s1;
        } else if (FREE && tx < 16 * 24 + 64) {
            const int x = tx - 16 * 24, r = x >> 2, col = x & 3;
            const float* al = sc_s + r * Ts;
            const float* ew = ew2_s + (int64_t)r * Ts * 4 + col;
            float s0 = 0.f, s1 = 0.f;
            int sp = 0;
            for (; sp + 1 < Ts; sp += 2) { s0 += al[sp] * ew[sp * 4]; s1 += al[sp + 1] * ew[(sp + 1) * 4]; }
            if (sp < Ts) s0 += al[sp] * ew[sp * 4];
            cw_s[x] = s0 + s1;
        }
        __syncthreads();
        if (eok) {
            float gi[3][4];
#pragma unroll
            for (int g = 0; g < 3; ++g) {
                const float4 x = *reinterpret_cast<const float4*>(gi_s + fr * 24 + g * 8 + 4 * hq);
                gi[g][0] = x.x; gi[g][1] = x.y; gi[g][2] = x.z; gi[g][3] = x.w;
            }
            float bi[3][4], hh[3][4];
#pragma unroll
            for (int g = 0; g < 3; ++g) {
                const float4 x = *reinterpret_cast<const float4*>(bs_s + 48 + g * 8 + 4 * hq);
                const float4 y = *reinterpret_cast<const float4*>(hp_s + fr * 24 + g * 8 + 4 * hq);
                bi[g][0] = x.x; bi[g][1] = x.y; bi[g][2] = x.z; bi[g][3] = x.w;
                hh[g][0] = y.x; hh[g][1] = y.y; hh[g][2] = y.z; hh[g][3] = y.w;
            }
            const float* hr = hh[0];
            const float* hz = hh[1];
            const float* hn = hh[2];
            const float4 h1v = *reinterpret_cast<const float4*>(hs_s + fr * 8 + 4 * hq);
            const float h1a[4] = {h1v.x, h1v.y, h1v.z, h1v.w};
            float rr[4], zz[4], nn[4], ho[4];
#pragma unroll
            for (int q = 0; q < 4; ++q) {
                rr[q] = vag_sigmoid(gi[0][q] + bi[0][q] + hr[q]);
                zz[q] = vag_sigmoid(gi[1][q] + bi[1][q] + hz[q]);
                nn[q] = vag_tanh(gi[2][q] + bi[2][q] + rr[q] * hn[q]);
                ho[q] = (1.f - zz[q]) * nn[q] + zz[q] * h1a[q];
            }
            const float4 h2v = tag4(make_float4(ho[0], ho[1], ho[2], ho[3]));
            *reinterpret_cast<float4*>(hs_s + 128 + fr * 8 + 4 * hq) = h2v;
            const int64_t o = (int64_t)em * H + eu;
            st_sc1_f4(a.h2_all + (int64_t)t * BH + o, h2v);
            if (!VAG_TAGGED) asm volatile("s_waitcnt vmcnt(0)" ::: "memory");
            if (VAG_TAGGED && tx == 0) arrive(c1 + t * CNT_WORDS, i);
            float* sv = a.g2 + (int64_t)t * 4 * BH + o;
            *reinterpret_cast<float4*>(sv) = make_float4(rr[0], rr[1], rr[2], rr[3]);
            *reinterpret_cast<float4*>(sv + BH) = make_float4(zz[0], zz[1], zz[2], zz[3]);
            *reinterpret_cast<float4*>(sv + 2 * BH) = make_float4(nn[0], nn[1], nn[2], nn[3]);
            *reinterpret_cast<float4*>(sv + 3 * BH) = make_float4(hn[0], hn[1], hn[2], hn[3]);
        }
        if (tx == 0 && (!VAG_TAGGED || !eok)) arrive(c1 + t * CNT_WORDS, i);
    }
#ifdef VAG_LAB
    if (!FREE && a.dbg && threadIdx.x == 0 && i == 0 && rt < 8) a.dbg[(Tt + 2) * 8 + rt] = __builtin_amdgcn_s_memrealtime();
#endif
#undef VAG_STAMP
}

struct DecBArgs {
    const float *pe, *encwp, *v, *wcatT, *whh1T;
    const float *h0, *h2_all, *h1, *g1, *g2, *qhp, *alpha;
    const float *d_h2_all, *dah;
    float *dgi2, *dqgh, *ds, *dgi1, *dgh1, *d_h0;
    float* dal;
    unsigned* cnt;
    unsigned* err;
    unsigned* guard;
    unsigned spin;
    unsigned long long* dbg;
    int B, Ts, Tt, H, RT;
    int rt0;
    int xcd_map;
    int h0_tanh;
    char *pl_dq, *pl_dgh1;
};

__device__ __forceinline__ void cell_bwd4(const float (&dh)[4], const float4 (&sv)[4], const float4 hp, float (&gi)[3][4],
                                          float (&gh)[3][4], float (&direct)[4]) {
    const float r_[4] = {sv[0].x, sv[0].y, sv[0].z, sv[0].w}, z_[4] = {sv[1].x, sv[1].y, sv[1].z, sv[1].w};
    const float n_[4] = {sv[2].x, sv[2].y, sv[2].z, sv[2].w}, hn[4] = {sv[3].x, sv[3].y, sv[3].z, sv[3].w};
    const float hpv[4] = {hp.x, hp.y, hp.z, hp.w};
#pragma unroll
    for (int q = 0; q < 4; ++q) {
        const float dn_pre = dh[q] * (1.f - z_[q]) * (1.f - n_[q] * n_[q]);
        const float dz_pre = dh[q] * (hpv[q] - n_[q]) * z_[q] * (1.f - z_[q]);
        const float dr_pre = dn_pre * hn[q] * r_[q] * (1.f - r_[q]);
        gi[0][q] = dr_pre; gi[1][q] = dz_pre; gi[2][q] = dn_pre;
        gh[0][q] = dr_pre; gh[1][q] = dz_pre; gh[2][q] = dn_pre * r_[q];
        direct[q] = dh[q] * z_[q];
    }
}

template <int WGS, bool PL>
__global__ __launch_bounds__(512, 1) void dec_bwd_persistent_kernel(DecBArgs a) {
    extern __shared__ __attribute__((aligned(16))) float dlds[];
    constexpr int H = WGS * DEC_U, C = 2 * H, Q = C + 3 * H;
    constexpr unsigned PER_SHARD = WGS / SHARDS;
    int i, rt;
    dec_slice_map<WGS>(a.xcd_map, a.rt0, i, rt);
    const int lane = threadIdx.x & 63, wave = threadIdx.x >> 6;
    const int B = a.B, Ts = a.Ts, Tt = a.Tt;
#ifdef VAG_LAB
#define VAG_BPSTAMP(k) do { if (a.dbg && blockIdx.x == 0 && threadIdx.x == 0) a.dbg[Tt * 8 + (k)] = __builtin_amdgcn_s_memrealtime(); } while (0)
#else
#define VAG_BPSTAMP(k) do { } while (0)
#endif
    VAG_BPSTAMP(0);
    const int m0 = rt * 16, u0 = i * DEC_U;
    const int fr = lane & 15, fg = lane >> 4;
    const int64_t BH = (int64_t)B * H;
    const int NP = 16 * Ts;
    float4* red = reinterpret_cast<float4*>(dlds);
    float* pe_s = dlds + 2048;
    float* ew_t = pe_s + NP * 16;
    float* da_s = ew_t + 24 * NP;
    float* al_s = da_s + NP;
    float* gi_s = al_s + NP;
    float* d1_s = gi_s + 384;
    float* pb_s = d1_s + 128;
    float* c1_s = pb_s + 128;
    float* dq_s = c1_s + 128;
    float* wb_s = dq_s + 256;
    constexpr int WBLD = C + 4;

    constexpr int KB = C / 8 / 32, KC = 3 * H / 8 / 32;
    bf16x8 wc[KC][3];
    {
        const float* pc = a.whh1T + (int64_t)(u0 + (fr & 7)) * (3 * H) + wave * (3 * H >> 3) + 8 * fg;
#pragma unroll
        for (int s = 0; s < KC; ++s) split8(*reinterpret_cast<const float4*>(pc + 32 * s), *reinterpret_cast<const float4*>(pc + 32 * s + 4), wc[s]);
    }
    for (int x = threadIdx.x; x < 8 * (C / 4); x += 512) {
        const int u = x / (C / 4), c4 = x - u * (C / 4);
        *reinterpret_cast<float4*>(wb_s + u * WBLD + 4 * c4) = *reinterpret_cast<const float4*>(a.wcatT + (int64_t)(u0 + u) * Q + 4 * c4);
    }
    const float* wb_row = wb_s + (fr & 7) * WBLD + wave * (C >> 3) + 8 * fg;
    const float* wa_row = a.wcatT + (int64_t)(u0 + (ld_row(lane) & 7)) * Q + C + wave * (3 * H >> 3) + 8 * (lane & 3);
    for (int x = threadIdx.x; x < NP * 4; x += 512) {
        const int P = x >> 2, c4 = x & 3;
        const int r = P / Ts, sp = P - r * Ts, b = min(m0 + r, B - 1);
        reinterpret_cast<float4*>(pe_s)[x] = *reinterpret_cast<const float4*>(a.pe + ((int64_t)b * Ts + sp) * C + 16 * i + 4 * c4);
    }
    for (int x = threadIdx.x; x < NP * 6; x += 512) {
        const int hf = x & 1, g = (x >> 1) % 3, P = x / 6;
        const int r = P / Ts, sp = P - r * Ts, b = min(m0 + r, B - 1);
        const float4 e = *reinterpret_cast<const float4*>(a.encwp + ((int64_t)b * Ts + sp) * 3 * H + g * H + u0 + 4 * hf);
        const int col = g * 8 + 4 * hf;
        ew_t[(col + 0) * NP + P] = e.x; ew_t[(col + 1) * NP + P] = e.y; ew_t[(col + 2) * NP + P] = e.z; ew_t[(col + 3) * NP + P] = e.w;
    }
    const int hq = (threadIdx.x >> 4) & 1;
    const int em = m0 + fr, eu = u0 + 4 * hq;
    const bool ep = threadIdx.x < 32, eok = ep && em < B;
    const int lrow = min(m0 + ld_row(lane), B - 1);
    const int src4 = ld_src4(lane);
    gu32* cA = (gu32*)(a.cnt + ((int64_t)0 * a.RT + rt) * Tt * CNT_WORDS);
    gu32* cB = (gu32*)(a.cnt + ((int64_t)1 * a.RT + rt) * Tt * CNT_WORDS);
    gu32* cC = (gu32*)(a.cnt + ((int64_t)2 * a.RT + rt) * Tt * CNT_WORDS);
    bool dead = false;
    const float vq = a.v[16 * i + (threadIdx.x & 15)];
    const char* pl_dq = PL ? a.pl_dq + (int64_t)rt * pl_block_bytes(C) : nullptr;
    const char* pl_g1 = PL ? a.pl_dgh1 + (int64_t)rt * pl_block_bytes(3 * H) : nullptr;
    const int64_t pl_dq_step = (int64_t)a.RT * pl_block_bytes(C), pl_g1_step = (int64_t)a.RT * pl_block_bytes(3 * H);
    const int pl_wave = __builtin_amdgcn_readfirstlane(wave) * PL_KSTEP_BYTES;
    constexpr int pl_gate = (H >> 5) * PL_KSTEP_BYTES;
    const int pl_st_g1 = (u0 >> 5) * PL_KSTEP_BYTES, pl_st_dq = ((16 * i) >> 5) * PL_KSTEP_BYTES;
    const unsigned pl_so_g1 = pl_slot_off(fr, eu), pl_so_dq = pl_slot_off((threadIdx.x >> 2) & 15, 16 * i + 4 * (threadIdx.x & 3));

    auto cell2_bwd = [&](int t, const float (&dh2)[4], const float4 (&sv)[4], const float4 hp) {
        float gi[3][4], gh[3][4], dr[4];
        cell_bwd4(dh2, sv, hp, gi, gh, dr);
#pragma unroll
        for (int g = 0; g < 3; ++g) {
            st_sc1_f4(a.dqgh + ((int64_t)t * B + em) * Q + C + g * H + eu, make_float4(gh[g][0], gh[g][1], gh[g][2], gh[g][3]));
            const float4 x = make_float4(gi[g][0], gi[g][1], gi[g][2], gi[g][3]);
            *reinterpret_cast<float4*>(gi_s + fr * 24 + g * 8 + 4 * hq) = x;
            *reinterpret_cast<float4*>(a.dgi2 + ((int64_t)t * B + em) * 3 * H + g * H + eu) = x;
        }
        *reinterpret_cast<float4*>(d1_s + fr * 8 + 4 * hq) = make_float4(dr[0], dr[1], dr[2], dr[3]);
    };
    auto red4 = [&](float (&x)[4]) {
        float4 sum = red[hq * 16 + fr];
#pragma unroll
        for (int w = 1; w < 8; ++w) {
            const float4 o = red[w * 64 + hq * 16 + fr];
            sum.x += o.x; sum.y += o.y; sum.z += o.z; sum.w += o.w;
        }
        x[0] = sum.x; x[1] = sum.y; x[2] = sum.z; x[3] = sum.w;
    };

    VAG_BPSTAMP(1);
    if (ep) {
        if (eok) {
            const float4 d = *reinterpret_cast<const float4*>(a.d_h2_all + (int64_t)(Tt - 1) * BH + (int64_t)em * H + eu);
            const float dh2[4] = {d.x, d.y, d.z, d.w};
            const int64_t o = (int64_t)em * H + eu;
            float4 sv[4];
#pragma unroll
            for (int q = 0; q < 4; ++q) sv[q] = *reinterpret_cast<const float4*>(a.g2 + ((int64_t)(Tt - 1) * 4 + q) * BH + o);
            cell2_bwd(Tt - 1, dh2, sv, *reinterpret_cast<const float4*>(a.h1 + (int64_t)(Tt - 1) * BH + o));
        } else {
#pragma unroll
            for (int g = 0; g < 3; ++g) *reinterpret_cast<float4*>(gi_s + fr * 24 + g * 8 + 4 * hq) = make_float4(0.f, 0.f, 0.f, 0.f);
            *reinterpret_cast<float4*>(d1_s + fr * 8 + 4 * hq) = make_float4(0.f, 0.f, 0.f, 0.f);
        }
    }
    __syncthreads();

#ifdef VAG_LAB
    const bool stamp = a.dbg != nullptr && blockIdx.x == 0 && threadIdx.x == 0;
#define VAG_STAMP(k) do { if (stamp) a.dbg[t * 8 + (k)] = __builtin_amdgcn_s_memrealtime(); } while (0)
#else
#define VAG_STAMP(k) do { } while (0)
#endif
    for (int t = Tt - 1; t >= 0; --t) {
        int emL = em;
        if (PL) asm volatile("" : "+v"(emL));
        VAG_STAMP(0);
        for (int P = threadIdx.x; P < NP; P += 512) {
            const int r = P / Ts;
            const float* g = gi_s + r * 24;
            float acc = 0.f;
#pragma unroll
            for (int k = 0; k < 24; ++k) acc += ew_t[k * NP + P] * g[k];
            if (m0 + r < B)
                atomicAdd(a.dal + (((int64_t)t * ACC_SHARDS + (i & (ACC_SHARDS - 1))) * B + m0 + r) * Ts + (P - r * Ts), acc);
        }
        asm volatile("s_waitcnt vmcnt(0)" ::: "memory");
        __syncthreads();
        if (threadIdx.x == 0) arrive(cA + t * CNT_WORDS, i);
        VAG_STAMP(1);
        float4 hga[KC], hgb[KC];
        static_assert(KC == 6 || KC == 3, "ld_acc_shards_and_rows<KC>");
        float al0 = 0.f, al1 = 0.f, dh0 = 0.f, dh1_ = 0.f;
        const int x0 = threadIdx.x, x1 = threadIdx.x + 512;
        {
            const int r0 = min(x0, NP - 1) / Ts, r1 = min(x1, NP - 1) / Ts;
            const int64_t o0 = ((int64_t)t * B + min(m0 + r0, B - 1)) * Ts + (min(x0, NP - 1) - r0 * Ts);
            const int64_t o1 = ((int64_t)t * B + min(m0 + r1, B - 1)) * Ts + (min(x1, NP - 1) - r1 * Ts);
            al0 = a.alpha[o0]; dh0 = a.dah[o0];
            if (x1 < NP) { al1 = a.alpha[o1]; dh1_ = a.dah[o1]; }
            const float qv = a.qhp[((int64_t)t * B + min(m0 + (int)((threadIdx.x & 255) >> 4), B - 1)) * Q + 16 * i + (threadIdx.x & 15)];
            wait_count(cA + t * CNT_WORDS, PER_SHARD, a.err, a.guard, a.spin, dead);
            VAG_STAMP(2);
            float v0, v1;
            const float* p0 = a.dal + o0 + (int64_t)t * (ACC_SHARDS - 1) * B * Ts;
            const float* p1 = a.dal + o1 + (int64_t)t * (ACC_SHARDS - 1) * B * Ts;
            ld_acc_shards_and_rows(p0, p1, (int64_t)B * Ts, v0, v1,
                                   a.dqgh + ((int64_t)t * B + lrow) * Q + C + wave * (3 * H >> 3) + 8 * (lane & 3), hga, hgb);
            if (x0 < NP) { da_s[x0] = v0 + dh0; al_s[x0] = al0; }
            if (x1 < NP) { da_s[x1] = v1 + dh1_; al_s[x1] = al1; }
            __syncthreads();
            for (int r = wave; r < 16; r += 8) {
                float dot = 0.f;
                for (int sp = lane; sp < Ts; sp += 64) dot += al_s[r * Ts + sp] * da_s[r * Ts + sp];
                dot = wave_sum(dot);
                for (int sp = lane; sp < Ts; sp += 64) {
                    const float d = al_s[r * Ts + sp] * (da_s[r * Ts + sp] - dot);
                    da_s[r * Ts + sp] = d;
                    if (((r * Ts + sp) & (WGS - 1)) == i && m0 + r < B) a.ds[((int64_t)t * B + m0 + r) * Ts + sp] = d;
                }
            }
            __syncthreads();
            {
                const int tt = threadIdx.x & 255, half = threadIdx.x >> 8;
                const int r = tt >> 4, c = tt & 15;
                const float* pr = pe_s + (int64_t)r * Ts * 16 + c;
                const float* dsr = da_s + r * Ts;
                float acc0 = 0.f, acc1 = 0.f;
                int sp = half;
                for (; sp + 2 < Ts; sp += 4) {
                    const float t0 = vag_tanh(pr[sp * 16] + qv), t1 = vag_tanh(pr[(sp + 2) * 16] + qv);
                    acc0 += dsr[sp] * (1.f - t0 * t0);
                    acc1 += dsr[sp + 2] * (1.f - t1 * t1);
                }
                if (sp < Ts) { const float t0 = vag_tanh(pr[sp * 16] + qv); acc0 += dsr[sp] * (1.f - t0 * t0); }
                float* half_s = reinterpret_cast<float*>(red);
                if (half) half_s[tt] = acc0 + acc1;
                __syncthreads();
                if (!half) dq_s[tt] = ((acc0 + acc1) + half_s[tt]) * vq;
            }
            __syncthreads();
            if (threadIdx.x < 64) {
                const int r = threadIdx.x >> 2, c4 = threadIdx.x & 3;
                const float4 dqv = *reinterpret_cast<const float4*>(dq_s + r * 16 + 4 * c4);
                float* dqo = a.dqgh + ((int64_t)t * B + m0 + r) * Q + 16 * i + 4 * c4;
                if (PL) st_planes4(pl_dq + t * pl_dq_step + pl_st_dq, pl_so_dq, m0 + r < B ? dqv : make_float4(0.f, 0.f, 0.f, 0.f));
                else if (m0 + r < B) st_sc1_f4(dqo, dqv);
                asm volatile("s_waitcnt vmcnt(0)" ::: "memory");
                if (threadIdx.x == 0) arrive(cB + t * CNT_WORDS, i);
                if (PL && m0 + r < B) *reinterpret_cast<float4*>(dqo) = dqv;
            }
        }
        VAG_STAMP(3);
        {
            f32x4 acc = {0.f, 0.f, 0.f, 0.f};
#pragma unroll
            for (int s = 0; s < KC; ++s) {
                bf16x8 wf[3], hf[3];
                split8(perm4(*reinterpret_cast<const float4*>(wa_row + 32 * s), src4),
                       perm4(*reinterpret_cast<const float4*>(wa_row + 32 * s + 4), src4), wf);
                split8(perm4(hga[s], src4), perm4(hgb[s], src4), hf);
                acc = mma6(wf, hf, acc);
            }
            red[wave * 64 + lane] = make_float4(acc[0], acc[1], acc[2], acc[3]);
            __syncthreads();
            if (ep) {
                float x[4];
                red4(x);
                const float4 d1 = *reinterpret_cast<const float4*>(d1_s + fr * 8 + 4 * hq);
                *reinterpret_cast<float4*>(pb_s + fr * 8 + 4 * hq) = make_float4(x[0] + d1.x, x[1] + d1.y, x[2] + d1.z, x[3] + d1.w);
            }
        }
        float4 s1[4], hp1 = make_float4(0.f, 0.f, 0.f, 0.f);
        if (eok) {
            const int64_t o = (int64_t)emL * H + eu;
#pragma unroll
            for (int q = 0; q < 4; ++q) s1[q] = *reinterpret_cast<const float4*>(a.g1 + ((int64_t)t * 4 + q) * BH + o);
            hp1 = *reinterpret_cast<const float4*>((t > 0 ? a.h2_all + (int64_t)(t - 1) * BH : a.h0) + o);
        }
        VAG_STAMP(4);
        wait_count(cB + t * CNT_WORDS, PER_SHARD, a.err, a.guard, a.spin, dead);
        VAG_STAMP(5);
        {
            f32x4 acc = {0.f, 0.f, 0.f, 0.f};
            if (PL) {
                u32x4 gf[3 * KB];
                ld_planes_sc1<KB>(pl_dq + t * pl_dq_step + KB * pl_wave, 16u * lane, gf);
#pragma unroll
                for (int s = 0; s < KB; ++s) {
                    bf16x8 wf[3];
                    split8(*reinterpret_cast<const float4*>(wb_row + 32 * s), *reinterpret_cast<const float4*>(wb_row + 32 * s + 4), wf);
                    const bf16x8 hf[3] = {__builtin_bit_cast(bf16x8, gf[3 * s]), __builtin_bit_cast(bf16x8, gf[3 * s + 1]),
                                          __builtin_bit_cast(bf16x8, gf[3 * s + 2])};
                    acc = mma6(wf, hf, acc);
                }
            } else {
                float4 ga[KB], gb[KB];
                ld_rows_sc1<KB>(a.dqgh + ((int64_t)t * B + lrow) * Q + wave * (C >> 3) + 8 * (lane & 3), ga, gb);
#pragma unroll
                for (int s = 0; s < KB; ++s) { ga[s] = perm4(ga[s], src4); gb[s] = perm4(gb[s], src4); }
#pragma unroll
                for (int s = 0; s < KB; ++s) {
                    bf16x8 wf[3], hf[3];
                    split8(*reinterpret_cast<const float4*>(wb_row + 32 * s), *reinterpret_cast<const float4*>(wb_row + 32 * s + 4), wf);
                    split8(ga[s], gb[s], hf);
                    acc = mma6(wf, hf, acc);
                }
            }
            red[wave * 64 + lane] = make_float4(acc[0], acc[1], acc[2], acc[3]);
        }
        __syncthreads();
        if (ep) {
            float x[4];
            red4(x);
            if (PL && !eok) {
#pragma unroll
                for (int g = 0; g < 3; ++g) st_planes4(pl_g1 + t * pl_g1_step + pl_st_g1 + g * pl_gate, pl_so_g1, make_float4(0.f, 0.f, 0.f, 0.f));
            }
            if (eok) {
                const float4 pbv = *reinterpret_cast<const float4*>(pb_s + fr * 8 + 4 * hq);
                const float dh1[4] = {x[0] + pbv.x, x[1] + pbv.y, x[2] + pbv.z, x[3] + pbv.w};
                float gi[3][4], gh[3][4], dr[4];
                cell_bwd4(dh1, s1, hp1, gi, gh, dr);
#pragma unroll
                for (int g = 0; g < 3; ++g) {
                    const float4 x = make_float4(gh[g][0], gh[g][1], gh[g][2], gh[g][3]);
                    if (PL) st_planes4(pl_g1 + t * pl_g1_step + pl_st_g1 + g * pl_gate, pl_so_g1, x);
                    else st_sc1_f4(a.dgh1 + ((int64_t)t * B + emL) * 3 * H + g * H + eu, x);
                }
                asm volatile("s_waitcnt vmcnt(0)" ::: "memory");
                if (threadIdx.x == 0) arrive(cC + t * CNT_WORDS, i);
#pragma unroll
                for (int g = 0; g < 3; ++g) {
                    if (PL)
                        *reinterpret_cast<float4*>(a.dgh1 + ((int64_t)t * B + emL) * 3 * H + g * H + eu) = make_float4(gh[g][0], gh[g][1], gh[g][2], gh[g][3]);
                    *reinterpret_cast<float4*>(a.dgi1 + ((int64_t)t * B + emL) * 3 * H + g * H + eu) = make_float4(gi[g][0], gi[g][1], gi[g][2], gi[g][3]);
                }
                *reinterpret_cast<float4*>(c1_s + fr * 8 + 4 * hq) = make_float4(dr[0], dr[1], dr[2], dr[3]);
            } else if (threadIdx.x == 0) {
                arrive(cC + t * CNT_WORDS, i);
            }
        }
        float4 dadd = make_float4(0.f, 0.f, 0.f, 0.f), s2[4], hp2 = make_float4(0.f, 0.f, 0.f, 0.f);
        if (eok && t > 0) {
            const int64_t o = (int64_t)emL * H + eu;
            dadd = *reinterpret_cast<const float4*>(a.d_h2_all + (int64_t)(t - 1) * BH + o);
#pragma unroll
            for (int q = 0; q < 4; ++q) s2[q] = *reinterpret_cast<const float4*>(a.g2 + ((int64_t)(t - 1) * 4 + q) * BH + o);
            hp2 = *reinterpret_cast<const float4*>(a.h1 + (int64_t)(t - 1) * BH + o);
        }
        VAG_STAMP(6);
        wait_count(cC + t * CNT_WORDS, PER_SHARD, a.err, a.guard, a.spin, dead);
        VAG_STAMP(7);
        {
            f32x4 acc = {0.f, 0.f, 0.f, 0.f};
            if (PL) {
                u32x4 gf[3 * KC];
                ld_planes_sc1<KC>(pl_g1 + t * pl_g1_step + KC * pl_wave, 16u * lane, gf);
                acc = mma6_planes<KC>(wc, gf, acc);
            } else {
                float4 ga[KC], gb[KC];
                ld_rows_sc1<KC>(a.dgh1 + ((int64_t)t * B + lrow) * 3 * H + wave * (3 * H >> 3) + 8 * (lane & 3), ga, gb);
#pragma unroll
                for (int s = 0; s < KC; ++s) { ga[s] = perm4(ga[s], src4); gb[s] = perm4(gb[s], src4); }
#pragma unroll
                for (int s = 0; s < KC; ++s) {
                    bf16x8 hf[3];
                    split8(ga[s], gb[s], hf);
                    acc = mma6(wc[s], hf, acc);
                }
            }
            red[wave * 64 + lane] = make_float4(acc[0], acc[1], acc[2], acc[3]);
        }
        __syncthreads();
        if (ep) {
            float x[4];
            red4(x);
            if (eok) {
                const float4 c1 = *reinterpret_cast<const float4*>(c1_s + fr * 8 + 4 * hq);
                const float dh2[4] = {x[0] + c1.x + dadd.x, x[1] + c1.y + dadd.y, x[2] + c1.z + dadd.z, x[3] + c1.w + dadd.w};
                if (t > 0) cell2_bwd(t - 1, dh2, s2, hp2);
                else {
                    float4 o = make_float4(dh2[0], dh2[1], dh2[2], dh2[3]);
                    if (a.h0_tanh) {
                        const float4 h = *reinterpret_cast<const float4*>(a.h0 + (int64_t)emL * H + eu);
                        o.x *= 1.f - h.x * h.x; o.y *= 1.f - h.y * h.y; o.z *= 1.f - h.z * h.z; o.w *= 1.f - h.w * h.w;
                    }
                    *reinterpret_cast<float4*>(a.d_h0 + (int64_t)emL * H + eu) = o;
                }
            }
        }
        __syncthreads();
    }
    VAG_BPSTAMP(2);
#undef VAG_STAMP
}

__global__ __launch_bounds__(256) void zero_u32_kernel(unsigned* p, int n) {
    const int i = blockIdx.x * 256 + threadIdx.x;
    if (i < n) p[i] = 0u;
}
__global__ __launch_bounds__(256) void zero2_u32_kernel(unsigned* p, int n, unsigned* q, int m) {
    const int i = blockIdx.x * 256 + threadIdx.x;
    if (i < n) p[i] = 0u;
    else if (i - n < m) q[i - n] = 0u;
}

}

struct PersistTimer { hipEvent_t e0 = nullptr, e1 = nullptr; bool pending = false; double ms = 0.0; int n = 0; };
static PersistTimer g_ptimer[4];
static std::mutex g_ptimer_mu;
static void ptimer_collect(PersistTimer& t) {
    if (!t.pending) return;
    float ms = 0.f;
    if (hipEventSynchronize(t.e1) == hipSuccess && hipEventElapsedTime(&ms, t.e0, t.e1) == hipSuccess) { t.ms += ms; ++t.n; }
    t.pending = false;
}
static bool ptimer_begin(int kind, hipStream_t s) {
    if (!vag_opt().persist_timing) return false;
    hipStreamCaptureStatus st = hipStreamCaptureStatusNone;
    if (hipStreamIsCapturing(s, &st) != hipSuccess) { (void)hipGetLastError(); return false; }
    if (st != hipStreamCaptureStatusNone) return false;
    std::lock_guard<std::mutex> lk(g_ptimer_mu);
    PersistTimer& t = g_ptimer[kind];
    ptimer_collect(t);
    if (!t.e0 && (hipEventCreate(&t.e0) != hipSuccess || hipEventCreate(&t.e1) != hipSuccess)) return false;
    return hipEventRecord(t.e0, s) == hipSuccess;
}
static void ptimer_end(int kind, hipStream_t s) {
    std::lock_guard<std::mutex> lk(g_ptimer_mu);
    if (hipEventRecord(g_ptimer[kind].e1, s) == hipSuccess) g_ptimer[kind].pending = true;
}
struct PTimerScope {
    const int kind;
    const hipStream_t s;
    const bool on;
    PTimerScope(int k, hipStream_t st) : kind(k), s(st), on(ptimer_begin(k, st)) {}
    ~PTimerScope() { if (on) ptimer_end(kind, s); }
};
int vag_persistent_time_read(int kind, double* ms_total, int* launches) {
    VAG_CHECK_ARG(kind >= 0 && kind < 4 && ms_total && launches);
    std::lock_guard<std::mutex> lk(g_ptimer_mu);
    PersistTimer& t = g_ptimer[kind];
    ptimer_collect(t);
    *ms_total = t.ms; *launches = t.n;
    t.ms = 0.0; t.n = 0;
    return VAG_OK;
}

struct PersistDev { std::atomic<int> cus{-1}; std::atomic<int> lds{-1}; };
static PersistDev g_pdev[64];
static PersistDev* persist_dev() {
    int dev = 0;
    if (hipGetDevice(&dev) != hipSuccess || dev < 0 || dev >= 64) return nullptr;
    PersistDev& d = g_pdev[dev];
    if (d.cus.load(std::memory_order_acquire) < 0) {
        int n = 0, l = 0;
        if (hipDeviceGetAttribute(&n, hipDeviceAttributeMultiprocessorCount, dev) != hipSuccess) n = 0;
        if (hipDeviceGetAttribute(&l, hipDeviceAttributeMaxSharedMemoryPerBlock, dev) != hipSuccess) l = 0;
        d.lds.store(l, std::memory_order_release);
        d.cus.store(n, std::memory_order_release);
    }
    return &d;
}
static int persist_cu_count() {
    PersistDev* d = persist_dev();
    return d ? d->cus.load(std::memory_order_acquire) : 0;
}
static bool persist_lds_ok(int64_t bytes) {
    PersistDev* d = persist_dev();
    return d && (int64_t)d->lds.load(std::memory_order_acquire) >= bytes;
}
static unsigned spin_limit() {
    const int64_t v = vag_opt().persist_spin_limit;
    return v > 0 ? (unsigned)(v > 0x7fffffff ? 0x7fffffff : v) : SPIN_LIMIT;
}
template <auto Kernel>
static bool max_lds_once() {
    static std::atomic<unsigned long long> done{0};
    int dev = 0;
    if (hipGetDevice(&dev) != hipSuccess || dev < 0 || dev >= 64) return false;
    const unsigned long long bit = 1ull << dev;
    if (done.load(std::memory_order_acquire) & bit) return true;
    if (hipFuncSetAttribute(reinterpret_cast<const void*>(Kernel), hipFuncAttributeMaxDynamicSharedMemorySize, 160 * 1024) != hipSuccess)
        return false;
    done.fetch_or(bit, std::memory_order_release);
    return true;
}
template <class Args>
static int sync_begin(Args& a, unsigned* sync, int64_t sync_words, hipStream_t s, float* acc = nullptr, int nacc = 0) {
    const int nwords = (int)sync_words;
    a.cnt = sync; a.err = sync + (nwords - 64); a.spin = spin_limit(); a.guard = vag_persist_guard();
    if (vag_ctx().persist_prezeroed) return VAG_OK;
    if (acc)
        hipLaunchKernelGGL(zero2_u32_kernel, dim3((unsigned)cdiv64((int64_t)nwords + nacc, 256)), dim3(256), 0, s, sync, nwords,
                           reinterpret_cast<unsigned*>(acc), nacc);
    else
        hipLaunchKernelGGL(zero_u32_kernel, dim3((unsigned)cdiv64(nwords, 256)), dim3(256), 0, s, sync, nwords);
    VAG_LAUNCH_CHECK();
    return VAG_OK;
}
template <class Launch>
static void row_tile_passes(int RT, int tpp, Launch&& launch) {
    for (int rt0 = 0; rt0 < RT; rt0 += tpp) launch(rt0, std::min(tpp, RT - rt0));
}
static int enc_tiles_per_pass(int64_t H) {
    const int cus = persist_cu_count();
    return (H == 256 || H == 512 || H == 1024) ? (int)(cus / (2 * (H / 16))) : 0;
}
static bool passes_ok(int64_t rt, int tpp, int max_passes) {
    if (tpp <= 0 || rt > (int64_t)tpp * max_passes) return false;
    return rt <= tpp || 4 * (rt - tpp * ((rt - 1) / tpp)) >= 3 * tpp;
}
bool vag_enc_persistent_ok(int64_t B, int64_t Ts, int64_t H) {
    if (!(H == 256 || H == 512 || H == 1024) || B <= 0 || Ts <= 0) return false;
    return passes_ok(cdiv64(B, 16), enc_tiles_per_pass(H), 2) && persist_lds_ok(84 * 1024) && (int64_t)(Ts + 1) * B * H * 4 < (1ll << 31);
}
int64_t vag_enc_persistent_sync_words(int64_t B, int64_t Ts) { return 2 * cdiv64(B, 16) * Ts + 64; }

int vag_enc_fwd_persistent_launch(const float* xp, const float* w_fw, const float* w_bw, const float* b_fw, const float* b_bw,
                                  const int* lengths, float* hst, float* gates, float* enc, unsigned* sync, const uint64_t* rng,
                                  float p_ctx, int64_t B, int64_t Ts, int64_t H, hipStream_t s) {
    VAG_CHECK_ARG(xp && w_fw && w_bw && b_fw && b_bw && lengths && hst && gates && enc && sync && vag_enc_persistent_ok(B, Ts, H));
    VAG_CHECK_ARG(aligned16(xp) && aligned16(w_fw) && aligned16(w_bw) && aligned16(b_fw) && aligned16(b_bw) && aligned16(hst) &&
                  aligned16(gates) && aligned16(enc));
    EncPArgs a;
    a.xp = xp; a.W[0] = w_fw; a.W[1] = w_bw; a.bias[0] = b_fw; a.bias[1] = b_bw; a.lengths = lengths;
    a.hst = hst; a.gates = gates; a.enc = enc; a.rng = rng; a.p_ctx = p_ctx;
    a.B = (int)B; a.Ts = (int)Ts; a.H = (int)H; a.RT = (int)cdiv64(B, 16); a.CS = (int)(H / 16);
    VAG_TRY(sync_begin(a, sync, vag_enc_persistent_sync_words(B, Ts), s));
    {
        PTimerScope timed(0, s);
        row_tile_passes(a.RT, enc_tiles_per_pass(H), [&](int rt0, int tiles) {
            a.rt0 = rt0; a.RTP = tiles;
            const dim3 grid((unsigned)(2 * a.RTP * a.CS));
            if (H == 256) hipLaunchKernelGGL(enc_fwd_persistent_kernel<1>, grid, dim3(512), 0, s, a);
            else if (H == 512) hipLaunchKernelGGL(enc_fwd_persistent_kernel<2>, grid, dim3(512), 0, s, a);
            else hipLaunchKernelGGL(enc_fwd_persistent_kernel<4>, grid, dim3(512), 0, s, a);
        });
    }
    VAG_LAUNCH_CHECK();
    return VAG_OK;
}

constexpr int DEC_MAX_PASSES = 2;
static int64_t dec_persistent_lds_bytes(int64_t Ts, bool free_run = false) {
    return 4 * (6144 + 16 * Ts * 16 + 16 * Ts * 24 + 16 * Ts + 16 * 24 + 16 * 24 + 80 + 256 + 1024 + 16 * Ts + 256 +
                (free_run ? 64 + 16 + 16 + 16 * Ts * 4 : 0));
}
static int dec_wgs(int64_t H) { return (int)(H / DEC_U); }
static int dec_tiles_per_pass(int64_t H) {
    const int cus = persist_cu_count();
    return (H == 256 || H == 512) ? cus / dec_wgs(H) : 0;
}
bool vag_dec_persistent_ok(int64_t B, int64_t Ts, int64_t Tt, int64_t H) {
    if ((H != 512 && H != 256) || B <= 0 || Ts <= 0 || Tt <= 0 || Ts > 512) return false;
    const int tpp = dec_tiles_per_pass(H);
    if (!passes_ok(cdiv64(B, 16), tpp, DEC_MAX_PASSES)) return false;
    return dec_persistent_lds_bytes(Ts) <= 160 * 1024 && persist_lds_ok(160 * 1024);
}
int64_t vag_dec_persistent_sync_words(int64_t B, int64_t Tt) { return 5 * cdiv64(B, 16) * Tt * CNT_WORDS + 64; }

static DecPArgs dec_fwd_args(const float* pe, const float* mask, const float* h0, const float* xp1, const float* W1, const float* b1,
                             const float* wcat, const float* bcat, const float* v, const float* encwp, const float* b_ih2, float* h1,
                             float* g1, float* qhp, float* alpha, float* h2_all, float* g2, float* psc, int64_t B, int64_t Ts,
                             int64_t Tt, int64_t H) {
    DecPArgs a = {};
    a.pe = pe; a.mask = mask; a.h0 = h0; a.xp1 = xp1; a.W1 = W1; a.b1 = b1; a.wcat = wcat; a.bcat = bcat; a.v = v; a.encwp = encwp;
    a.b_ih2 = b_ih2; a.h1 = h1; a.g1 = g1; a.qhp = qhp; a.alpha = alpha; a.h2_all = h2_all; a.g2 = g2; a.psc = psc;
    a.B = (int)B; a.Ts = (int)Ts; a.Tt = (int)Tt; a.H = (int)H; a.RT = (int)cdiv64(B, 16);
    a.xcd_map = vag_opt().dec_xcd_map & 15;
#ifdef VAG_LAB
    a.dbg = reinterpret_cast<unsigned long long*>(vag_opt().dec_stamps);
#else
    a.dbg = nullptr;
#endif
    return a;
}
static int dec_fwd_zero(DecPArgs& a, unsigned* sync, hipStream_t s) {
    VAG_TRY(sync_begin(a, sync, vag_dec_persistent_sync_words(a.B, a.Tt), s, a.psc, a.Tt * a.B * a.Ts * ACC_SHARDS));
    if (VAG_TAGGED && !vag_ctx().persist_prezeroed) {
        const int nh = a.Tt * a.B * a.H;
        hipLaunchKernelGGL(zero2_u32_kernel, dim3((unsigned)cdiv64(2 * (int64_t)nh, 256)), dim3(256), 0, s,
                           reinterpret_cast<unsigned*>(a.h1), nh, reinterpret_cast<unsigned*>(a.h2_all), nh);
        VAG_LAUNCH_CHECK();
    }
    return VAG_OK;
}

int vag_dec_fwd_persistent_launch(const float* pe, const float* mask, const float* h0, const float* xp1, const float* W1,
                                  const float* b1, const float* wcat, const float* bcat, const float* v, const float* encwp,
                                  const float* b_ih2, float* h1, float* g1, float* qhp, float* alpha, float* h2_all, float* g2,
                                  float* psc, unsigned* sync, int64_t B, int64_t Ts, int64_t Tt, int64_t H, hipStream_t s) {
    VAG_CHECK_ARG(pe && mask && h0 && xp1 && W1 && b1 && wcat && bcat && v && encwp && b_ih2 && h1 && g1 && qhp && alpha && h2_all &&
                  g2 && psc && sync && vag_dec_persistent_ok(B, Ts, Tt, H));
    VAG_CHECK_ARG(aligned16(pe) && aligned16(h0) && aligned16(xp1) && aligned16(W1) && aligned16(b1) && aligned16(wcat) &&
                  aligned16(bcat) && aligned16(v) && aligned16(encwp) && aligned16(b_ih2) && aligned16(h1) && aligned16(g1) &&
                  aligned16(qhp) && aligned16(h2_all) && aligned16(g2));
    DecPArgs a = dec_fwd_args(pe, mask, h0, xp1, W1, b1, wcat, bcat, v, encwp, b_ih2, h1, g1, qhp, alpha, h2_all, g2, psc, B, Ts, Tt, H);
    VAG_TRY(dec_fwd_zero(a, sync, s));
    int64_t lds = dec_persistent_lds_bytes(Ts);
    if (lds < 84 * 1024) lds = 84 * 1024;
    if (!max_lds_once<dec_fwd_persistent_kernel<false, 64>>()) return VAG_EINVAL;
    if (H == 256 && !max_lds_once<dec_fwd_persistent_kernel<false, 32>>()) return VAG_EINVAL;
    {
        PTimerScope timed(1, s);
        row_tile_passes(a.RT, dec_tiles_per_pass(H), [&](int rt0, int tiles) {
            a.rt0 = rt0;
            if (H == 512) hipLaunchKernelGGL((dec_fwd_persistent_kernel<false, 64>), dim3(tiles * 64u), dim3(512), (size_t)lds, s, a);
            else hipLaunchKernelGGL((dec_fwd_persistent_kernel<false, 32>), dim3(tiles * 32u), dim3(512), (size_t)lds, s, a);
        });
    }
    VAG_LAUNCH_CHECK();
    return VAG_OK;
}

bool vag_dec_free_persistent_ok(int64_t B, int64_t Ts, int64_t Tt, int64_t E, int64_t H, int64_t V) {
    if (H != 512 || E != DEC_E || B <= 0 || B > 64 || Ts <= 0 || Tt <= 0 || Ts > 512 || V < 16 || V >= (1ll << 30)) return false;
    const int cus = persist_cu_count();
    return cdiv64(B, 16) * DEC_WGS <= cus && dec_persistent_lds_bytes(Ts, true) <= 160 * 1024 && persist_lds_ok(160 * 1024);
}
// ... 14 lines not shown
                                   int64_t H, int64_t V, hipStream_t s) {
    const float* tables = tab.embp;
    VAG_CHECK_ARG(pe && mask && h0 && W1 && b1 && wcat && bcat && v && encwp && b_ih2 && h1 && g1 && qhp && alpha && h2_all && g2 &&
                  psc && sync && tables && hw1 && hb1 && hb2 && hb3 && out_w && out_b && tmid && tok &&
                  vag_dec_free_persistent_ok(B, Ts, Tt, E, H, V));
    VAG_CHECK_ARG(aligned16(pe) && aligned16(h0) && aligned16(W1) && aligned16(b1) && aligned16(wcat) && aligned16(bcat) &&
                  aligned16(v) && aligned16(encwp) && aligned16(b_ih2) && aligned16(h1) && aligned16(g1) && aligned16(qhp) &&
                  aligned16(h2_all) && aligned16(g2) && aligned16(tables) && aligned16(hw1) && aligned16(out_w) && aligned16(tmid));
    VAG_CHECK_ARG(!logits || (aligned16(logits) && ldl >= V && ldl % 4 == 0));
    DecPArgs a = dec_fwd_args(pe, mask, h0, nullptr, W1, b1, wcat, bcat, v, encwp, b_ih2, h1, g1, qhp, alpha, h2_all, g2, psc, B, Ts, Tt, H);
    a.embp = tab.embp; a.embw3 = tab.embw3; a.encw2 = tab.encw2; a.cand = tab.cand;
    a.hw1 = hw1; a.hb1 = hb1; a.hb2 = hb2; a.hb3 = hb3; a.out_w = out_w; a.out_b = out_b; a.tmid = tmid; a.logits = logits;
    a.tok = tok; a.rng = rng; a.p_out = p_out; a.V = (int)V; a.ldl = (int)ldl;
    VAG_TRY(dec_fwd_zero(a, sync, s));
    int64_t lds = dec_persistent_lds_bytes(Ts, true);
    if (lds < 84 * 1024) lds = 84 * 1024;
    if (!max_lds_once<dec_fwd_persistent_kernel<true>>()) return VAG_EINVAL;
    {
        PTimerScope timed(1, s);
        hipLaunchKernelGGL(dec_fwd_persistent_kernel<true>, dim3((unsigned)(a.RT * DEC_WGS)), dim3(512), (size_t)lds, s, a);
    }
    VAG_LAUNCH_CHECK();
    return VAG_OK;
}

bool vag_enc_wide16_ok(int64_t B, int64_t Ts, int64_t H) {
    if (!(H == 512 || H == 1024) || B < 1 || Ts < 1) return false;
    const int64_t wgs = 2 * cdiv64(B, 64) * (H / 32);
    if (wgs > persist_cu_count() || !persist_lds_ok(160 * 1024)) return false;
    return 2 * cdiv64(B, 64) * Ts + 64 <= vag_enc_persistent_sync_words(B, Ts);
}
int vag_enc_fwd_wide16_launch(const float* xp, const vag_half* w16_fw, const vag_half* w16_bw, const float* b_fw, const float* b_bw,
                              const int* lengths, float* hst, float* gates, float* enc, vag_half* hx, unsigned* sync, const uint64_t* rng,
                              float p_ctx, int64_t B, int64_t Ts, int64_t H, hipStream_t s) {
    VAG_CHECK_ARG(xp && w16_fw && w16_bw && b_fw && b_bw && lengths && hst && gates && enc && hx && sync &&
                  vag_enc_wide16_ok(B, Ts, H));
    VAG_CHECK_ARG(aligned16(xp) && aligned16(w16_fw) && aligned16(w16_bw) && aligned16(b_fw) && aligned16(b_bw) && aligned16(hst) &&
                  aligned16(gates) && aligned16(enc) && aligned16(hx));
    EncWArgs a;
    a.xp = xp; a.W16[0] = w16_fw; a.W16[1] = w16_bw; a.bias[0] = b_fw; a.bias[1] = b_bw; a.lengths = lengths;
    a.hst = hst; a.gates = gates; a.enc = enc; a.hx = hx; a.rng = rng; a.p_ctx = p_ctx;
    a.B = (int)B; a.Ts = (int)Ts; a.H = (int)H; a.RG = (int)cdiv64(B, 64); a.CS = (int)(H / 32);
    VAG_TRY(sync_begin(a, sync, vag_enc_persistent_sync_words(B, Ts), s));
    const size_t lds = 96 * 1024;
    if (!max_lds_once<enc_fwd_wide16_kernel<4>>() || !max_lds_once<enc_fwd_wide16_kernel<8>>()) return VAG_EINVAL;
    const dim3 grid((unsigned)(2 * a.RG * a.CS));
    {
        PTimerScope timed(0, s);
        if (H == 512) hipLaunchKernelGGL(enc_fwd_wide16_kernel<4>, grid, dim3(512), lds, s, a);
        else hipLaunchKernelGGL(enc_fwd_wide16_kernel<8>, grid, dim3(512), lds, s, a);
    }
    VAG_LAUNCH_CHECK();
    return VAG_OK;
}

int vag_enc_bwd_wide16_launch(const vag_half* wt16, const float* d_enc, const float* gates, const float* hst, const int* lengths,
                              const uint64_t* rng, float p_ctx, float* d_xp, float* dgh, vag_half* gx, unsigned* sync, int64_t B,
                              int64_t Ts, int64_t H, hipStream_t s) {
    VAG_CHECK_ARG(wt16 && d_enc && gates && hst && lengths && d_xp && dgh && gx && sync && vag_enc_wide16_ok(B, Ts, H));
    VAG_CHECK_ARG(aligned16(wt16) && aligned16(d_enc) && aligned16(gates) && aligned16(hst) && aligned16(d_xp) && aligned16(dgh) &&
                  aligned16(gx));
    EncWBArgs a;
    a.WT16[0] = wt16; a.WT16[1] = wt16 + 3 * H * H; a.d_enc = d_enc; a.gates = gates; a.hst = hst; a.lengths = lengths;
    a.rng = rng; a.p_ctx = p_ctx; a.d_xp = d_xp; a.dgh = dgh; a.gx = gx;
    a.B = (int)B; a.Ts = (int)Ts; a.H = (int)H; a.RG = (int)cdiv64(B, 64); a.CS = (int)(H / 32);
    VAG_TRY(sync_begin(a, sync, vag_enc_persistent_sync_words(B, Ts), s));
    const size_t lds = 84 * 1024;
    if (!max_lds_once<enc_bwd_wide16_kernel<6>>() || !max_lds_once<enc_bwd_wide16_kernel<12>>()) return VAG_EINVAL;
    const dim3 grid((unsigned)(2 * a.RG * a.CS));
    {
        PTimerScope timed(2, s);
        if (H == 512) hipLaunchKernelGGL(enc_bwd_wide16_kernel<6>, grid, dim3(512), lds, s, a);
        else hipLaunchKernelGGL(enc_bwd_wide16_kernel<12>, grid, dim3(512), lds, s, a);
    }
    VAG_LAUNCH_CHECK();
    return VAG_OK;
}

int vag_enc_bwd_persistent_launch(const float* whhT, const float* d_enc, const float* gates, const float* hst, const int* lengths,
                                  const uint64_t* rng, float p_ctx, float* d_xp, float* dgh, float* planes, unsigned* sync, int64_t B,
                                  int64_t Ts, int64_t H, hipStream_t s) {
    VAG_CHECK_ARG(whhT && d_enc && gates && hst && lengths && d_xp && dgh && sync && (H == 512 || H == 256) && vag_enc_persistent_ok(B, Ts, H));
    VAG_CHECK_ARG(aligned16(whhT) && aligned16(d_enc) && aligned16(gates) && aligned16(hst) && aligned16(d_xp) && aligned16(dgh) && aligned16(planes));
    const bool pl = planes && vag_opt().handoff_planes && vag_enc_bwd_planes_floats(B, Ts, H) > 0;
    EncBArgs a;
    a.WT[0] = whhT; a.WT[1] = whhT + 3 * H * H; a.d_enc = d_enc; a.gates = gates; a.hst = hst; a.lengths = lengths;
    a.rng = rng; a.p_ctx = p_ctx; a.d_xp = d_xp; a.dgh = dgh; a.pl = reinterpret_cast<char*>(planes);
    a.B = (int)B; a.Ts = (int)Ts; a.H = (int)H; a.RT = (int)cdiv64(B, 16); a.CS = (int)(H / 16);
    VAG_TRY(sync_begin(a, sync, vag_enc_persistent_sync_words(B, Ts), s));
    {
        PTimerScope timed(2, s);
        row_tile_passes(a.RT, enc_tiles_per_pass(H), [&](int rt0, int tiles) {
            a.rt0 = rt0; a.RTP = tiles;
            const dim3 grid((unsigned)(2 * a.RTP * a.CS));
            if (H == 512 && pl) hipLaunchKernelGGL((enc_bwd_persistent_kernel<6, true>), grid, dim3(512), 0, s, a);
            else if (H == 512) hipLaunchKernelGGL((enc_bwd_persistent_kernel<6, false>), grid, dim3(512), 0, s, a);
            else if (pl) hipLaunchKernelGGL((enc_bwd_persistent_kernel<3, true>), grid, dim3(512), 0, s, a);
            else hipLaunchKernelGGL((enc_bwd_persistent_kernel<3, false>), grid, dim3(512), 0, s, a);
        });
    }
    VAG_LAUNCH_CHECK();
    return VAG_OK;
}

unsigned* vag_persist_guard(void) {
    if (vag_ctx().guard) return vag_ctx().guard;
    void* p = nullptr;
    if (hipGetSymbolAddress(&p, HIP_SYMBOL(g_persist_guard)) != hipSuccess) { (void)hipGetLastError(); return nullptr; }
    return reinterpret_cast<unsigned*>(p);
}
int vag_persistent_timeouts_read(void) {
    unsigned v = 0, z = 0;
    const unsigned zz[2] = {0u, 0u};
    if (hipMemcpyFromSymbol(&v, HIP_SYMBOL(g_persist_timeouts), sizeof(v)) != hipSuccess) return -1;
    if (v != 0 && (hipMemcpyToSymbol(HIP_SYMBOL(g_persist_timeouts), &z, sizeof(z)) != hipSuccess ||
                   hipMemcpyToSymbol(HIP_SYMBOL(g_persist_guard), zz, sizeof(zz)) != hipSuccess)) return -1;
    return (int)v;
}

static int64_t dec_bwd_persistent_lds_bytes(int64_t Ts, int64_t H = 512) {
    const int64_t NP = 16 * Ts;
    return 4 * (2048 + NP * 16 + 24 * NP + 2 * NP + 384 + 3 * 128 + 256 + 8 * (2 * H + 4) + 64);
}
static bool pl_any_device_takes(int64_t rt, int tpp_max) {
    for (int tpp = 1; tpp <= tpp_max; ++tpp)
        if (passes_ok(rt, tpp, DEC_MAX_PASSES)) return true;
    return false;
}
constexpr int PL_MAX_CUS = 256;
int64_t vag_enc_bwd_planes_floats(int64_t B, int64_t Ts, int64_t H) {
    if ((H != 512 && H != 256) || B <= 0 || Ts <= 0 || !pl_any_device_takes(cdiv64(B, 16), (int)(PL_MAX_CUS / (2 * (H / 16))))) return 0;
    return 2 * Ts * cdiv64(B, 16) * pl_block_bytes(3 * H) / 4;
}
int64_t vag_dec_bwd_planes_floats(int64_t B, int64_t Tt, int64_t H) {
    if ((H != 512 && H != 256) || B <= 0 || Tt <= 0 || !pl_any_device_takes(cdiv64(B, 16), PL_MAX_CUS / dec_wgs(H))) return 0;
    return Tt * cdiv64(B, 16) * (pl_block_bytes(2 * H) + pl_block_bytes(3 * H)) / 4;
}
bool vag_dec_bwd_persistent_ok(int64_t B, int64_t Ts, int64_t Tt, int64_t H) {
    return vag_dec_persistent_ok(B, Ts, Tt, H) && dec_bwd_persistent_lds_bytes(Ts, H) <= 160 * 1024;
}
int vag_dec_bwd_persistent_launch(const float* pe, const float* encwp, const float* v, const float* wcatT, const float* whh1T,
                                  const float* h0, const float* h2_all, const float* h1, const float* g1, const float* g2,
                                  const float* qhp, const float* alpha, const float* d_h2_all, const float* dah, float* dgi2,
                                  float* dqgh, float* ds, float* dgi1, float* dgh1, float* d_h0, float* dal, float* planes,
                                  unsigned* sync, int64_t B, int64_t Ts, int64_t Tt, int64_t H, hipStream_t s) {
    VAG_CHECK_ARG(pe && encwp && v && wcatT && whh1T && h0 && h2_all && h1 && g1 && g2 && qhp && alpha && d_h2_all && dah && dgi2 &&
                  dqgh && ds && dgi1 && dgh1 && d_h0 && dal && sync && vag_dec_bwd_persistent_ok(B, Ts, Tt, H));
    VAG_CHECK_ARG(aligned16(pe) && aligned16(encwp) && aligned16(wcatT) && aligned16(whh1T) && aligned16(h0) && aligned16(h2_all) &&
                  aligned16(h1) && aligned16(g1) && aligned16(g2) && aligned16(qhp) && aligned16(d_h2_all) && aligned16(dgi2) &&
                  aligned16(dqgh) && aligned16(dgi1) && aligned16(dgh1) && aligned16(d_h0) && aligned16(planes));
    const bool pl = planes && vag_opt().handoff_planes && vag_dec_bwd_planes_floats(B, Tt, H) > 0;
    DecBArgs a;
    a.pe = pe; a.encwp = encwp; a.v = v; a.wcatT = wcatT; a.whh1T = whh1T; a.h0 = h0; a.h2_all = h2_all; a.h1 = h1; a.g1 = g1;
    a.g2 = g2; a.qhp = qhp; a.alpha = alpha; a.d_h2_all = d_h2_all; a.dah = dah; a.dgi2 = dgi2; a.dqgh = dqgh; a.ds = ds;
    a.dgi1 = dgi1; a.dgh1 = dgh1; a.d_h0 = d_h0; a.dal = dal;
    VagCallCtx::Dh0Tanh& dh0 = vag_ctx().dh0_tanh;
    a.h0_tanh = dh0.req ? 1 : 0;
    if (dh0.req) dh0.done = d_h0;
    dh0.req = false;
#ifdef VAG_LAB
    a.dbg = reinterpret_cast<unsigned long long*>(vag_opt().dec_bwd_stamps);
#else
    a.dbg = nullptr;
#endif
    a.B = (int)B; a.Ts = (int)Ts; a.Tt = (int)Tt; a.H = (int)H; a.RT = (int)cdiv64(B, 16);
    a.pl_dq = reinterpret_cast<char*>(planes);
    a.pl_dgh1 = a.pl_dq ? a.pl_dq + Tt * a.RT * pl_block_bytes(2 * H) : nullptr;
    a.xcd_map = vag_opt().dec_xcd_map >> 4;
    VAG_TRY(sync_begin(a, sync, vag_dec_persistent_sync_words(B, Tt), s, dal, (int)(Tt * B * Ts) * ACC_SHARDS));
    int64_t lds = dec_bwd_persistent_lds_bytes(Ts, H);
    if (lds < 84 * 1024) lds = 84 * 1024;
    if (H == 512 && !(pl ? max_lds_once<dec_bwd_persistent_kernel<64, true>>() : max_lds_once<dec_bwd_persistent_kernel<64, false>>())) return VAG_EINVAL;
    if (H == 256 && !(pl ? max_lds_once<dec_bwd_persistent_kernel<32, true>>() : max_lds_once<dec_bwd_persistent_kernel<32, false>>())) return VAG_EINVAL;
    {
        PTimerScope timed(3, s);
        row_tile_passes(a.RT, dec_tiles_per_pass(H), [&](int rt0, int tiles) {
            a.rt0 = rt0;
            if (H == 512 && pl) hipLaunchKernelGGL((dec_bwd_persistent_kernel<64, true>), dim3(tiles * 64u), dim3(512), (size_t)lds, s, a);
            else if (H == 512) hipLaunchKernelGGL((dec_bwd_persistent_kernel<64, false>), dim3(tiles * 64u), dim3(512), (size_t)lds, s, a);
            else if (pl) hipLaunchKernelGGL((dec_bwd_persistent_kernel<32, true>), dim3(tiles * 32u), dim3(512), (size_t)lds, s, a);
            else hipLaunchKernelGGL((dec_bwd_persistent_kernel<32, false>), dim3(tiles * 32u), dim3(512), (size_t)lds, s, a);
        });
    }
    VAG_LAUNCH_CHECK();
    return VAG_OK;
}
```

Measured before the change: 22350 sentence-pairs/s.

## Extend bf16 hand-off planes to encoder forward and decoder-backward hidden side

The encoder forward persistent kernel now publishes each step's hidden state as pre-split bf16 planes, so consumer waves load MMA-ready fragments instead of loading fp32 rows and permuting and splitting them. The decoder backward persistent kernel gains a mode that writes the hidden-side dgh2 gradients into planes and caches pre-split recurrent weights in a per-workgroup plane buffer. The aim is to shorten the cross-workgroup critical path in the serial recurrences. In exchange the shared handoff buffer grows and extra writes are added, since fp32 copies are still stored for later consumers.

```diff
diff --git a/vag-nmt_amd/csrc/api.hip b/vag-nmt_amd/csrc/api.hip
--- a/vag-nmt_amd/csrc/api.hip
+++ b/vag-nmt_amd/csrc/api.hip
@@ -151,8 +151,9 @@
     const bool s16 = vag_ctx().store16 && vag_ctx().derived;
     VAG_CHECK_ARG(!vag_ctx().store16 || (vag_ctx().derived && H % 8 == 0));
     if (!s16 && vag_opt().persistent && vag_enc_persistent_ok(B, Ts, H)) {
-        return vag_enc_fwd_persistent_launch(w.xp, fw.w_hh, bw.w_hh, fw.b_hh, bw.b_hh, lengths, w.hst, w.gates, enc, w.sync, rng,
-                                             p_ctx, B, Ts, H, s);
+        return vag_enc_fwd_persistent_launch(w.xp, fw.w_hh, bw.w_hh, fw.b_hh, bw.b_hh, lengths, w.hst, w.gates, enc,
+                                             vag_ctx().handoff_planes, vag_ctx().handoff_planes ? vag_ctx().handoff_floats : 0, w.sync,
+                                             rng, p_ctx, B, Ts, H, s);
     }
     const vag_half* w16 = s16 ? derived_layout(const_cast<float*>(vag_ctx().derived), H).enc16 : nullptr;
     if (s16 && vag_opt().persistent && vag_enc_wide16_ok(B, Ts, H) && B >= 64) {
@@ -700,7 +701,8 @@
     if (persist) {
         VAG_TRY(vag_dec_bwd_persistent_launch(pe, k.encwp, w.attn_v, z.wcatT, z.whh1T, h0, h2_all, k.h1, k.g1, k.g2, k.qhp, k.alpha,
                                               d_h2_all, z.dah, z.dgi2, z.dqgh, z.ds, z.dgi1, z.dgh1, d_h0, k.dal,
-                                              handoff_planes(vag_dec_bwd_planes_floats(B, Tt, H)), k.sync_b, B, Ts, Tt, H, s));
+                                              vag_ctx().handoff_planes, vag_ctx().handoff_planes ? vag_ctx().handoff_floats : 0,
+                                              k.sync_b, B, Ts, Tt, H, s));
     }
     for (int64_t t = Tt - 1; t >= 0 && !persist; --t) {
         float* dgi2 = z.dgi2 + t * B * 3 * H;
@@ -1430,8 +1432,8 @@
 }
 int vag_persistent_timeouts(void) { return vag_persistent_timeouts_read(); }
 int64_t vag_handoff_planes_floats(int64_t B, int64_t Ts, int64_t Tt, int64_t H) {
-    const int64_t e = vag_enc_bwd_planes_floats(B, Ts, H), d = vag_dec_bwd_planes_floats(B, Tt, H);
-    return e > d ? e : d;
+    const int64_t e = vag_enc_bwd_planes_floats(B, Ts, H), d = vag_dec_bwd_planes_floats(B, Tt, H), f = vag_enc_fwd_planes_floats(B, Ts, H);
+    return std::max(std::max(e, d), f);
 }
 int vag_set_handoff_planes(float* buf, int64_t floats) {
     VAG_CHECK_ARG((buf == nullptr || (floats > 0 && aligned16(buf))));
diff --git a/vag-nmt_amd/csrc/common.h b/vag-nmt_amd/csrc/common.h
--- a/vag-nmt_amd/csrc/common.h
+++ b/vag-nmt_amd/csrc/common.h
@@ -102,7 +102,7 @@
     int persistent_dec_bwd = 1;
     int persistent_enc_bwd = 1;
     int attn_dot_reg = 1;
-    int handoff_planes = 1;
+    int handoff_planes = 7;
     int free_persistent = 1;
     int s16_one_plane = 1;
     int head_bf16_dlogits = 1;
diff --git a/vag-nmt_amd/csrc/kernels.h b/vag-nmt_amd/csrc/kernels.h
--- a/vag-nmt_amd/csrc/kernels.h
+++ b/vag-nmt_amd/csrc/kernels.h
@@ -169,8 +169,9 @@
 bool vag_enc_persistent_ok(int64_t B, int64_t Ts, int64_t H);
 int64_t vag_enc_persistent_sync_words(int64_t B, int64_t Ts);
 int vag_enc_fwd_persistent_launch(const float* xp, const float* w_fw, const float* w_bw, const float* b_fw, const float* b_bw,
-                                  const int* lengths, float* hst, float* gates, float* enc, unsigned* sync, const uint64_t* rng,
-                                  float p_ctx, int64_t B, int64_t Ts, int64_t H, hipStream_t s);
+                                  const int* lengths, float* hst, float* gates, float* enc, float* planes, int64_t planes_floats,
+                                  unsigned* sync, const uint64_t* rng, float p_ctx, int64_t B, int64_t Ts, int64_t H, hipStream_t s);
+int64_t vag_enc_fwd_planes_floats(int64_t B, int64_t Ts, int64_t H);
 int vag_enc_bwd_persistent_launch(const float* whhT, const float* d_enc, const float* gates, const float* hst, const int* lengths,
                                   const uint64_t* rng, float p_ctx, float* d_xp, float* dgh, float* planes, unsigned* sync, int64_t B,
                                   int64_t Ts, int64_t H, hipStream_t s);
@@ -195,7 +196,7 @@
                                   const float* h0, const float* h2_all, const float* h1, const float* g1, const float* g2,
                                   const float* qhp, const float* alpha, const float* d_h2_all, const float* dah, float* dgi2,
                                   float* dqgh, float* ds, float* dgi1, float* dgh1, float* d_h0, float* dal, float* planes,
-                                  unsigned* sync, int64_t B, int64_t Ts, int64_t Tt, int64_t H, hipStream_t s);
+                                  int64_t planes_floats, unsigned* sync, int64_t B, int64_t Ts, int64_t Tt, int64_t H, hipStream_t s);
 float* vag_cgru_bwd_scratch_de(float* scratch, int64_t B, int64_t Ts, int64_t Tt, int64_t E, int64_t H);
 float* vag_cgru_bwd_scratch_du(float* scratch, int64_t B, int64_t Ts, int64_t Tt, int64_t E, int64_t H);
 int vag_attn_dot_row_launch(bool bwd, const float* x, const float* q, int64_t ldq, const float* mask, const float* alpha, int64_t B,
diff --git a/vag-nmt_amd/csrc/persist.hip b/vag-nmt_amd/csrc/persist.hip
--- a/vag-nmt_amd/csrc/persist.hip
+++ b/vag-nmt_amd/csrc/persist.hip
@@ -35,6 +35,7 @@
     float p_ctx;
     int B, Ts, H, RT, CS;
     int rt0, RTP;
+    char* pl;
 };
 
 template <int N> __device__ __forceinline__ void ld_rows_sc1(const float* p, float4 (&a)[N], float4 (&b)[N]);
@@ -146,6 +147,8 @@
 
 constexpr int PL_PLANE_BYTES = 64 * 16, PL_KSTEP_BYTES = 3 * PL_PLANE_BYTES;
 __host__ __device__ constexpr int64_t pl_block_bytes(int64_t K) { return (K / 32) * PL_KSTEP_BYTES; }
+constexpr int PL_W2_PLANE_BYTES = 32 * 16, PL_W2_KSTEP_BYTES = 3 * PL_W2_PLANE_BYTES;
+__host__ __device__ constexpr int64_t pl_w2_bytes(int64_t H) { return (3 * H / 32) * PL_W2_KSTEP_BYTES; }
 typedef unsigned u32x2 __attribute__((ext_vector_type(2)));
 __device__ __forceinline__ unsigned pl_slot_off(int r, int k0) { return (unsigned)((r + 16 * ((k0 & 31) >> 3)) * 16 + 8 * ((k0 >> 2) & 1)); }
 __device__ __forceinline__ void st_planes4(const char* kblk, unsigned voff, float4 v) {
@@ -159,6 +162,11 @@
 }
 #define VAG_PLD(o, v, a, off) "global_load_dwordx4 %" #o ", %" #v ", %" #a " offset:" #off " sc1\n\t"
 template <int N> __device__ __forceinline__ void ld_planes_sc1(const char* p, unsigned voff, u32x4 (&f)[3 * N]);
+template <> __device__ __forceinline__ void ld_planes_sc1<1>(const char* p, unsigned voff, u32x4 (&f)[3]) {
+    asm volatile(VAG_PLD(0, 3, 4, 0) VAG_PLD(1, 3, 4, 1024) VAG_PLD(2, 3, 4, 2048)
+                 "s_waitcnt vmcnt(0)"
+                 : "=&v"(f[0]), "=&v"(f[1]), "=&v"(f[2]) : "v"(voff), "s"(p) : "memory");
+}
 template <> __device__ __forceinline__ void ld_planes_sc1<2>(const char* p, unsigned voff, u32x4 (&f)[6]) {
     const char* p1 = p + 8192;
     asm volatile(VAG_PLD(0, 6, 7, 0) VAG_PLD(1, 6, 7, 1024) VAG_PLD(2, 6, 7, 2048) VAG_PLD(3, 6, 7, 3072) VAG_PLD(4, 6, 8, -4096) VAG_PLD(5, 6, 8, -3072)
@@ -206,7 +214,7 @@
     return acc;
 }
 
-template <int KS>
+template <int KS, bool PL>
 __global__ __launch_bounds__(512, 1) void enc_fwd_persistent_kernel(EncPArgs a) {
     __shared__ __attribute__((aligned(16))) float lds[21504];
     const int wg = blockIdx.x;
@@ -249,6 +257,10 @@
     const int src4 = ld_src4(lane);
     float4* red = reinterpret_cast<float4*>(lds);
     bool dead = false;
+    const char* pld = PL ? a.pl + ((int64_t)d * Ts * a.RT + rt) * pl_block_bytes(H) : nullptr;
+    const int64_t pl_step = (int64_t)a.RT * pl_block_bytes(H);
+    const int pl_ld = __builtin_amdgcn_readfirstlane(wave) * (KS * PL_KSTEP_BYTES), pl_st = (u0 >> 5) * PL_KSTEP_BYTES;
+    const unsigned pl_so = pl_slot_off(erow, eu);
 
     for (int k = 0; k < Ts; ++k) {
         const int t = d == 0 ? k : Ts - 1 - k;
@@ -268,19 +280,36 @@
             __syncthreads();
         }
         f32x4 acc[3] = {{0.f, 0.f, 0.f, 0.f}, {0.f, 0.f, 0.f, 0.f}, {0.f, 0.f, 0.f, 0.f}};
-        float4 h0[KS], h1[KS];
-        if (k > 0) {
-            ld_rows_sc1<KS>(hs + ((int64_t)k * B + lrow) * H + kbase + 8 * (lane & 3), h0, h1);
+        if constexpr (PL) {
+            u32x4 gf[3 * KS];
+            if (k > 0) {
+                ld_planes_sc1<KS>(pld + (k - 1) * pl_step + pl_ld, 16u * lane, gf);
+            } else {
+#pragma unroll
+                for (int s = 0; s < 3 * KS; ++s) gf[s] = u32x4{0u, 0u, 0u, 0u};
+            }
+#pragma unroll
+            for (int s = 0; s < KS; ++s) {
+                const bf16x8 hf[3] = {__builtin_bit_cast(bf16x8, gf[3 * s]), __builtin_bit_cast(bf16x8, gf[3 * s + 1]),
+                                      __builtin_bit_cast(bf16x8, gf[3 * s + 2])};
+#pragma unroll
+                for (int j = 0; j < 3; ++j) acc[j] = mma6(wf[s][j], hf, acc[j]);
+            }
         } else {
-#pragma unroll
-            for (int s = 0; s < KS; ++s) h0[s] = h1[s] = make_float4(0.f, 0.f, 0.f, 0.f);
-        }
-#pragma unroll
-        for (int s = 0; s < KS; ++s) {
-            bf16x8 hf[3];
-            split8(perm4(h0[s], src4), perm4(h1[s], src4), hf);
-#pragma unroll
-            for (int j = 0; j < 3; ++j) acc[j] = mma6(wf[s][j], hf, acc[j]);
+            float4 h0[KS], h1[KS];
+            if (k > 0) {
+                ld_rows_sc1<KS>(hs + ((int64_t)k * B + lrow) * H + kbase + 8 * (lane & 3), h0, h1);
+            } else {
+#pragma unroll
+                for (int s = 0; s < KS; ++s) h0[s] = h1[s] = make_float4(0.f, 0.f, 0.f, 0.f);
+            }
+#pragma unroll
+            for (int s = 0; s < KS; ++s) {
+                bf16x8 hf[3];
+                split8(perm4(h0[s], src4), perm4(h1[s], src4), hf);
+#pragma unroll
+                for (int j = 0; j < 3; ++j) acc[j] = mma6(wf[s][j], hf, acc[j]);
+            }
         }
 #pragma unroll
         for (int j = 0; j < 3; ++j) red[(wave * 3 + j) * 64 + lane] = make_float4(acc[j][0], acc[j][1], acc[j][2], acc[j][3]);
@@ -297,6 +326,7 @@
                 }
                 c[j] = make_float4(sum.x + bb[j].x, sum.y + bb[j].y, sum.z + bb[j].z, sum.w + bb[j].w);
             }
+            if (PL && !eok) st_planes4(pld + k * pl_step + pl_st, pl_so, make_float4(0.f, 0.f, 0.f, 0.f));
             if (eok) {
                 const bool active = t < len;
                 const float cr[4] = {c[0].x, c[0].y, c[0].z, c[0].w}, cz[4] = {c[1].x, c[1].y, c[1].z, c[1].w};
@@ -316,9 +346,11 @@
                 }
                 hp = make_float4(ho[0], ho[1], ho[2], ho[3]);
                 const int64_t o = (int64_t)em * H + eu;
-                st_sc1(rs, (unsigned)((((int64_t)(k + 1) * B) * H + o) * 4), hp);
+                if (PL) st_planes4(pld + k * pl_step + pl_st, pl_so, hp);
+                else st_sc1(rs, (unsigned)((((int64_t)(k + 1) * B) * H + o) * 4), hp);
                 asm volatile("s_waitcnt vmcnt(0)" ::: "memory");
                 if (lane == 0) __hip_atomic_fetch_add(cnt + k, 1u, RLX_AGENT);
+                if (PL) *reinterpret_cast<float4*>(hs + ((int64_t)(k + 1) * B) * H + o) = hp;
                 float* sv = a.gates + ((int64_t)(d * Ts + k) * 4) * BH + o;
                 *reinterpret_cast<float4*>(sv) = make_float4(rr[0], rr[1], rr[2], rr[3]);
                 *reinterpret_cast<float4*>(sv + BH) = make_float4(zz[0], zz[1], zz[2], zz[3]);
@@ -1491,6 +1523,7 @@
     int xcd_map;
     int h0_tanh;
     char *pl_dq, *pl_dgh1;
+    char *pl_dgh2, *pl_w2;
 };
 
 __device__ __forceinline__ void cell_bwd4(const float (&dh)[4], const float4 (&sv)[4], const float4 hp, float (&gi)[3][4],
@@ -1509,9 +1542,11 @@
     }
 }
 
-template <int WGS, bool PL>
+template <int WGS, int PLM>
 __global__ __launch_bounds__(512, 1) void dec_bwd_persistent_kernel(DecBArgs a) {
     extern __shared__ __attribute__((aligned(16))) float dlds[];
+    constexpr bool PL = (PLM & 1) != 0, PL2 = (PLM & 2) != 0;
+    static_assert(PL || !PL2, "the hidden side's planes come with the hand-off planes");
     constexpr int H = WGS * DEC_U, C = 2 * H, Q = C + 3 * H;
     constexpr unsigned PER_SHARD = WGS / SHARDS;
     int i, rt;
@@ -1554,6 +1589,22 @@
     }
     const float* wb_row = wb_s + (fr & 7) * WBLD + wave * (C >> 3) + 8 * fg;
     const float* wa_row = a.wcatT + (int64_t)(u0 + (ld_row(lane) & 7)) * Q + C + wave * (3 * H >> 3) + 8 * (lane & 3);
+    const char* pl_w2 = PL2 ? a.pl_w2 + (int64_t)blockIdx.x * pl_w2_bytes(H) + __builtin_amdgcn_readfirstlane(wave) * (KC * PL_W2_KSTEP_BYTES) : nullptr;
+    const unsigned pl_w2_off = (unsigned)(((fr & 7) + 8 * fg) * 16);
+    if (PL2) {
+        const float* pw = a.wcatT + (int64_t)(u0 + (fr & 7)) * Q + C + wave * (3 * H >> 3) + 8 * fg;
+#pragma unroll
+        for (int s = 0; s < KC; ++s) {
+            bf16x8 wf[3];
+            split8(*reinterpret_cast<const float4*>(pw + 32 * s), *reinterpret_cast<const float4*>(pw + 32 * s + 4), wf);
+            if (fr < 8) {
+#pragma unroll
+                for (int p = 0; p < 3; ++p)
+                    *reinterpret_cast<bf16x8*>(const_cast<char*>(pl_w2) + pl_w2_off + s * PL_W2_KSTEP_BYTES + p * PL_W2_PLANE_BYTES) = wf[p];
+            }
+        }
+        asm volatile("s_waitcnt vmcnt(0)" ::: "memory");
+    }
     for (int x = threadIdx.x; x < NP * 4; x += 512) {
         const int P = x >> 2, c4 = x & 3;
         const int r = P / Ts, sp = P - r * Ts, b = min(m0 + r, B - 1);
@@ -1578,18 +1629,22 @@
     const float vq = a.v[16 * i + (threadIdx.x & 15)];
     const char* pl_dq = PL ? a.pl_dq + (int64_t)rt * pl_block_bytes(C) : nullptr;
     const char* pl_g1 = PL ? a.pl_dgh1 + (int64_t)rt * pl_block_bytes(3 * H) : nullptr;
+    const char* pl_g2 = PL2 ? a.pl_dgh2 + (int64_t)rt * pl_block_bytes(3 * H) : nullptr;
     const int64_t pl_dq_step = (int64_t)a.RT * pl_block_bytes(C), pl_g1_step = (int64_t)a.RT * pl_block_bytes(3 * H);
     const int pl_wave = __builtin_amdgcn_readfirstlane(wave) * PL_KSTEP_BYTES;
     constexpr int pl_gate = (H >> 5) * PL_KSTEP_BYTES;
     const int pl_st_g1 = (u0 >> 5) * PL_KSTEP_BYTES, pl_st_dq = ((16 * i) >> 5) * PL_KSTEP_BYTES;
     const unsigned pl_so_g1 = pl_slot_off(fr, eu), pl_so_dq = pl_slot_off((threadIdx.x >> 2) & 15, 16 * i + 4 * (threadIdx.x & 3));
 
+    float4 gh2k[3] = {make_float4(0.f, 0.f, 0.f, 0.f), make_float4(0.f, 0.f, 0.f, 0.f), make_float4(0.f, 0.f, 0.f, 0.f)};
     auto cell2_bwd = [&](int t, const float (&dh2)[4], const float4 (&sv)[4], const float4 hp) {
         float gi[3][4], gh[3][4], dr[4];
         cell_bwd4(dh2, sv, hp, gi, gh, dr);
 #pragma unroll
         for (int g = 0; g < 3; ++g) {
-            st_sc1_f4(a.dqgh + ((int64_t)t * B + em) * Q + C + g * H + eu, make_float4(gh[g][0], gh[g][1], gh[g][2], gh[g][3]));
+            const float4 y = make_float4(gh[g][0], gh[g][1], gh[g][2], gh[g][3]);
+            if (PL2) { st_planes4(pl_g2 + t * pl_g1_step + pl_st_g1 + g * pl_gate, pl_so_g1, y); gh2k[g] = y; }
+            else st_sc1_f4(a.dqgh + ((int64_t)t * B + em) * Q + C + g * H + eu, y);
             const float4 x = make_float4(gi[g][0], gi[g][1], gi[g][2], gi[g][3]);
             *reinterpret_cast<float4*>(gi_s + fr * 24 + g * 8 + 4 * hq) = x;
             *reinterpret_cast<float4*>(a.dgi2 + ((int64_t)t * B + em) * 3 * H + g * H + eu) = x;
@@ -1604,6 +1659,17 @@
             sum.x += o.x; sum.y += o.y; sum.z += o.z; sum.w += o.w;
         }
         x[0] = sum.x; x[1] = sum.y; x[2] = sum.z; x[3] = sum.w;
+    };
+    auto hid_load = [&](int t, int c, bf16x8 (&wf)[3][3], u32x4 (&gf)[9]) {
+        unsigned w2o = pl_w2_off;
+        asm volatile("" : "+v"(w2o));
+        const char* pw = pl_w2 + w2o;
+#pragma unroll
+        for (int s = 0; s < 3; ++s)
+#pragma unroll
+            for (int p = 0; p < 3; ++p)
+                wf[s][p] = *reinterpret_cast<const bf16x8*>(pw + (3 * c + s) * PL_W2_KSTEP_BYTES + p * PL_W2_PLANE_BYTES);
+        ld_planes_sc1<3>(pl_g2 + t * pl_g1_step + KC * pl_wave + c * (3 * PL_KSTEP_BYTES), 16u * lane, gf);
     };
 
     VAG_BPSTAMP(1);
@@ -1620,6 +1686,10 @@
 #pragma unroll
             for (int g = 0; g < 3; ++g) *reinterpret_cast<float4*>(gi_s + fr * 24 + g * 8 + 4 * hq) = make_float4(0.f, 0.f, 0.f, 0.f);
             *reinterpret_cast<float4*>(d1_s + fr * 8 + 4 * hq) = make_float4(0.f, 0.f, 0.f, 0.f);
+            if (PL2) {
+#pragma unroll
+                for (int g = 0; g < 3; ++g) st_planes4(pl_g2 + (Tt - 1) * pl_g1_step + pl_st_g1 + g * pl_gate, pl_so_g1, make_float4(0.f, 0.f, 0.f, 0.f));
+            }
         }
     }
     __syncthreads();
@@ -1646,9 +1716,15 @@
         asm volatile("s_waitcnt vmcnt(0)" ::: "memory");
         __syncthreads();
         if (threadIdx.x == 0) arrive(cA + t * CNT_WORDS, i);
+        if (PL2 && eok) {
+#pragma unroll
+            for (int g = 0; g < 3; ++g) *reinterpret_cast<float4*>(a.dqgh + ((int64_t)t * B + emL) * Q + C + g * H + eu) = gh2k[g];
+        }
         VAG_STAMP(1);
-        float4 hga[KC], hgb[KC];
-        static_assert(KC == 6 || KC == 3, "ld_acc_shards_and_rows<KC>");
+        float4 hga[PL2 ? 1 : KC], hgb[PL2 ? 1 : KC];
+        bf16x8 wf0[3][3];
+        u32x4 gf0[9];
+        static_assert(KC == 6 || KC == 3, "ld_acc_shards_and_rows<KC>, chunks of three k-steps");
         float al0 = 0.f, al1 = 0.f, dh0 = 0.f, dh1_ = 0.f;
         const int x0 = threadIdx.x, x1 = threadIdx.x + 512;
         {
@@ -1663,8 +1739,9 @@
             float v0, v1;
             const float* p0 = a.dal + o0 + (int64_t)t * (ACC_SHARDS - 1) * B * Ts;
             const float* p1 = a.dal + o1 + (int64_t)t * (ACC_SHARDS - 1) * B * Ts;
-            ld_acc_shards_and_rows(p0, p1, (int64_t)B * Ts, v0, v1,
-                                   a.dqgh + ((int64_t)t * B + lrow) * Q + C + wave * (3 * H >> 3) + 8 * (lane & 3), hga, hgb);
+            if constexpr (PL2) ld_acc_shards(p0, p1, (int64_t)B * Ts, v0, v1);
+            else ld_acc_shards_and_rows(p0, p1, (int64_t)B * Ts, v0, v1,
+                                        a.dqgh + ((int64_t)t * B + lrow) * Q + C + wave * (3 * H >> 3) + 8 * (lane & 3), hga, hgb);
             if (x0 < NP) { da_s[x0] = v0 + dh0; al_s[x0] = al0; }
             if (x1 < NP) { da_s[x1] = v1 + dh1_; al_s[x1] = al1; }
             __syncthreads();
@@ -1698,7 +1775,18 @@
                 if (!half) dq_s[tt] = ((acc0 + acc1) + half_s[tt]) * vq;
             }
             __syncthreads();
-            if (threadIdx.x < 64) {
+            if constexpr (PL2) {
+                const int r = (threadIdx.x >> 2) & 15, c4 = threadIdx.x & 3;
+                const bool w0 = threadIdx.x < 64;
+                float4 dqv = make_float4(0.f, 0.f, 0.f, 0.f);
+                if (w0) {
+                    dqv = *reinterpret_cast<const float4*>(dq_s + r * 16 + 4 * c4);
+                    st_planes4(pl_dq + t * pl_dq_step + pl_st_dq, pl_so_dq, m0 + r < B ? dqv : make_float4(0.f, 0.f, 0.f, 0.f));
+                }
+                hid_load(t, 0, wf0, gf0);
+                if (threadIdx.x == 0) arrive(cB + t * CNT_WORDS, i);
+                if (w0 && m0 + r < B) *reinterpret_cast<float4*>(a.dqgh + ((int64_t)t * B + m0 + r) * Q + 16 * i + 4 * c4) = dqv;
+            } else if (threadIdx.x < 64) {
                 const int r = threadIdx.x >> 2, c4 = threadIdx.x & 3;
                 const float4 dqv = *reinterpret_cast<const float4*>(dq_s + r * 16 + 4 * c4);
                 float* dqo = a.dqgh + ((int64_t)t * B + m0 + r) * Q + 16 * i + 4 * c4;
@@ -1712,13 +1800,22 @@
         VAG_STAMP(3);
         {
             f32x4 acc = {0.f, 0.f, 0.f, 0.f};
-#pragma unroll
-            for (int s = 0; s < KC; ++s) {
-                bf16x8 wf[3], hf[3];
-                split8(perm4(*reinterpret_cast<const float4*>(wa_row + 32 * s), src4),
-                       perm4(*reinterpret_cast<const float4*>(wa_row + 32 * s + 4), src4), wf);
-                split8(perm4(hga[s], src4), perm4(hgb[s], src4), hf);
-                acc = mma6(wf, hf, acc);
+            if constexpr (PL2) {
+                acc = mma6_planes<3>(wf0, gf0, acc);
+#pragma unroll
+                for (int c = 1; c < KC / 3; ++c) {
+                    hid_load(t, c, wf0, gf0);
+                    acc = mma6_planes<3>(wf0, gf0, acc);
+                }
+            } else {
+#pragma unroll
+                for (int s = 0; s < KC; ++s) {
+                    bf16x8 wf[3], hf[3];
+                    split8(perm4(*reinterpret_cast<const float4*>(wa_row + 32 * s), src4),
+                           perm4(*reinterpret_cast<const float4*>(wa_row + 32 * s + 4), src4), wf);
+                    split8(perm4(hga[s], src4), perm4(hgb[s], src4), hf);
+                    acc = mma6(wf, hf, acc);
+                }
             }
             red[wave * 64 + lane] = make_float4(acc[0], acc[1], acc[2], acc[3]);
             __syncthreads();
@@ -1831,11 +1928,15 @@
             red[wave * 64 + lane] = make_float4(acc[0], acc[1], acc[2], acc[3]);
         }
         __syncthreads();
+        if (PL2) {
+#pragma unroll
+            for (int g = 0; g < 3; ++g) gh2k[g] = make_float4(0.f, 0.f, 0.f, 0.f);
+        }
         if (ep) {
             float x[4];
             red4(x);
             if (eok) {
-                const float4 c1 = *reinterpret_cast<const float4*>(c1_s + fr * 8 + 4 * hq);
+                const float4 c1 =*reinterpret_cast<const float4*>(c1_s + fr * 8 + 4 * hq);
                 const float dh2[4] = {x[0] + c1.x + dadd.x, x[1] + c1.y + dadd.y, x[2] + c1.z + dadd.z, x[3] + c1.w + dadd.w};
                 if (t > 0) cell2_bwd(t - 1, dh2, s2, hp2);
                 else {
@@ -1846,6 +1947,9 @@
                     }
                     *reinterpret_cast<float4*>(a.d_h0 + (int64_t)emL * H + eu) = o;
                 }
+            } else if (PL2 && t > 0) {
+#pragma unroll
+                for (int g = 0; g < 3; ++g) st_planes4(pl_g2 + (t - 1) * pl_g1_step + pl_st_g1 + g * pl_gate, pl_so_g1, make_float4(0.f, 0.f, 0.f, 0.f));
             }
         }
         __syncthreads();
@@ -1978,12 +2082,15 @@
 int64_t vag_enc_persistent_sync_words(int64_t B, int64_t Ts) { return 2 * cdiv64(B, 16) * Ts + 64; }
 
 int vag_enc_fwd_persistent_launch(const float* xp, const float* w_fw, const float* w_bw, const float* b_fw, const float* b_bw,
-                                  const int* lengths, float* hst, float* gates, float* enc, unsigned* sync, const uint64_t* rng,
-                                  float p_ctx, int64_t B, int64_t Ts, int64_t H, hipStream_t s) {
+                                  const int* lengths, float* hst, float* gates, float* enc, float* planes, int64_t planes_floats,
+                                  unsigned* sync, const uint64_t* rng, float p_ctx, int64_t B, int64_t Ts, int64_t H, hipStream_t s) {
     VAG_CHECK_ARG(xp && w_fw && w_bw && b_fw && b_bw && lengths && hst && gates && enc && sync && vag_enc_persistent_ok(B, Ts, H));
     VAG_CHECK_ARG(aligned16(xp) && aligned16(w_fw) && aligned16(w_bw) && aligned16(b_fw) && aligned16(b_bw) && aligned16(hst) &&
-                  aligned16(gates) && aligned16(enc));
+                  aligned16(gates) && aligned16(enc) && aligned16(planes));
+    const int64_t pl_need = vag_enc_fwd_planes_floats(B, Ts, H);
+    const bool pl = planes && (vag_opt().handoff_planes & 4) && pl_need > 0 && planes_floats >= pl_need;
     EncPArgs a;
+    a.pl = pl ? reinterpret_cast<char*>(planes) : nullptr;
     a.xp = xp; a.W[0] = w_fw; a.W[1] = w_bw; a.bias[0] = b_fw; a.bias[1] = b_bw; a.lengths = lengths;
     a.hst = hst; a.gates = gates; a.enc = enc; a.rng = rng; a.p_ctx = p_ctx;
     a.B = (int)B; a.Ts = (int)Ts; a.H = (int)H; a.RT = (int)cdiv64(B, 16); a.CS = (int)(H / 16);
@@ -1993,9 +2100,12 @@
         row_tile_passes(a.RT, enc_tiles_per_pass(H), [&](int rt0, int tiles) {
             a.rt0 = rt0; a.RTP = tiles;
             const dim3 grid((unsigned)(2 * a.RTP * a.CS));
-            if (H == 256) hipLaunchKernelGGL(enc_fwd_persistent_kernel<1>, grid, dim3(512), 0, s, a);
-            else if (H == 512) hipLaunchKernelGGL(enc_fwd_persistent_kernel<2>, grid, dim3(512), 0, s, a);
-            else hipLaunchKernelGGL(enc_fwd_persistent_kernel<4>, grid, dim3(512), 0, s, a);
+            if (H == 256 && pl) hipLaunchKernelGGL((enc_fwd_persistent_kernel<1, true>), grid, dim3(512), 0, s, a);
+            else if (H == 256) hipLaunchKernelGGL((enc_fwd_persistent_kernel<1, false>), grid, dim3(512), 0, s, a);
+            else if (H == 512 && pl) hipLaunchKernelGGL((enc_fwd_persistent_kernel<2, true>), grid, dim3(512), 0, s, a);
+            else if (H == 512) hipLaunchKernelGGL((enc_fwd_persistent_kernel<2, false>), grid, dim3(512), 0, s, a);
+            else if (pl) hipLaunchKernelGGL((enc_fwd_persistent_kernel<4, true>), grid, dim3(512), 0, s, a);
+            else hipLaunchKernelGGL((enc_fwd_persistent_kernel<4, false>), grid, dim3(512), 0, s, a);
         });
     }
     VAG_LAUNCH_CHECK();
@@ -2176,7 +2286,7 @@
                                   int64_t Ts, int64_t H, hipStream_t s) {
     VAG_CHECK_ARG(whhT && d_enc && gates && hst && lengths && d_xp && dgh && sync && (H == 512 || H == 256) && vag_enc_persistent_ok(B, Ts, H));
     VAG_CHECK_ARG(aligned16(whhT) && aligned16(d_enc) && aligned16(gates) && aligned16(hst) && aligned16(d_xp) && aligned16(dgh) && aligned16(planes));
-    const bool pl = planes && vag_opt().handoff_planes && vag_enc_bwd_planes_floats(B, Ts, H) > 0;
+    const bool pl = planes && (vag_opt().handoff_planes & 1) && vag_enc_bwd_planes_floats(B, Ts, H) > 0;
     EncBArgs a;
     a.WT[0] = whhT; a.WT[1] = whhT + 3 * H * H; a.d_enc = d_enc; a.gates = gates; a.hst = hst; a.lengths = lengths;
     a.rng = rng; a.p_ctx = p_ctx; a.d_xp = d_xp; a.dgh = dgh; a.pl = reinterpret_cast<char*>(planes);
@@ -2226,9 +2336,21 @@
     if ((H != 512 && H != 256) || B <= 0 || Ts <= 0 || !pl_any_device_takes(cdiv64(B, 16), (int)(PL_MAX_CUS / (2 * (H / 16))))) return 0;
     return 2 * Ts * cdiv64(B, 16) * pl_block_bytes(3 * H) / 4;
 }
-int64_t vag_dec_bwd_planes_floats(int64_t B, int64_t Tt, int64_t H) {
+int64_t vag_enc_fwd_planes_floats(int64_t B, int64_t Ts, int64_t H) {
+    if ((H != 1024 && H != 512 && H != 256) || B <= 0 || Ts <= 0 || !pl_any_device_takes(cdiv64(B, 16), (int)(PL_MAX_CUS / (2 * (H / 16))))) return 0;
+    return 2 * Ts * cdiv64(B, 16) * pl_block_bytes(H) / 4;
+}
+static int64_t dec_bwd_handoff_floats(int64_t B, int64_t Tt, int64_t H) {
     if ((H != 512 && H != 256) || B <= 0 || Tt <= 0 || !pl_any_device_takes(cdiv64(B, 16), PL_MAX_CUS / dec_wgs(H))) return 0;
     return Tt * cdiv64(B, 16) * (pl_block_bytes(2 * H) + pl_block_bytes(3 * H)) / 4;
+}
+static int64_t dec_bwd_hidden_floats(int64_t B, int64_t Tt, int64_t H, int64_t tiles_per_pass) {
+    const int64_t RT = cdiv64(B, 16);
+    return (Tt * RT * pl_block_bytes(3 * H) + std::min(RT, tiles_per_pass) * dec_wgs(H) * pl_w2_bytes(H)) / 4;
+}
+int64_t vag_dec_bwd_planes_floats(int64_t B, int64_t Tt, int64_t H) {
+    const int64_t base = dec_bwd_handoff_floats(B, Tt, H);
+    return base > 0 ? base + dec_bwd_hidden_floats(B, Tt, H, PL_MAX_CUS / dec_wgs(H)) : 0;
 }
 bool vag_dec_bwd_persistent_ok(int64_t B, int64_t Ts, int64_t Tt, int64_t H) {
     return vag_dec_persistent_ok(B, Ts, Tt, H) && dec_bwd_persistent_lds_bytes(Ts, H) <= 160 * 1024;
@@ -2237,13 +2359,17 @@
                                   const float* h0, const float* h2_all, const float* h1, const float* g1, const float* g2,
                                   const float* qhp, const float* alpha, const float* d_h2_all, const float* dah, float* dgi2,
                                   float* dqgh, float* ds, float* dgi1, float* dgh1, float* d_h0, float* dal, float* planes,
-                                  unsigned* sync, int64_t B, int64_t Ts, int64_t Tt, int64_t H, hipStream_t s) {
+                                  int64_t planes_floats, unsigned* sync, int64_t B, int64_t Ts, int64_t Tt, int64_t H, hipStream_t s) {
     VAG_CHECK_ARG(pe && encwp && v && wcatT && whh1T && h0 && h2_all && h1 && g1 && g2 && qhp && alpha && d_h2_all && dah && dgi2 &&
                   dqgh && ds && dgi1 && dgh1 && d_h0 && dal && sync && vag_dec_bwd_persistent_ok(B, Ts, Tt, H));
     VAG_CHECK_ARG(aligned16(pe) && aligned16(encwp) && aligned16(wcatT) && aligned16(whh1T) && aligned16(h0) && aligned16(h2_all) &&
                   aligned16(h1) && aligned16(g1) && aligned16(g2) && aligned16(qhp) && aligned16(d_h2_all) && aligned16(dgi2) &&
                   aligned16(dqgh) && aligned16(dgi1) && aligned16(dgh1) && aligned16(d_h0) && aligned16(planes));
-    const bool pl = planes && vag_opt().handoff_planes && vag_dec_bwd_planes_floats(B, Tt, H) > 0;
+    const int64_t pl_base = dec_bwd_handoff_floats(B, Tt, H);
+    const int64_t pl_hid = dec_bwd_hidden_floats(B, Tt, H, dec_tiles_per_pass(H));
+    const int plopt = vag_opt().handoff_planes;
+    const bool pl = planes && (plopt & 1) && pl_base > 0 && planes_floats >= pl_base;
+    const bool pl2 = pl && (plopt & 2) && planes_floats >= vag_dec_bwd_planes_floats(B, Tt, H) && planes_floats >= pl_base + pl_hid;
     DecBArgs a;
     a.pe = pe; a.encwp = encwp; a.v = v; a.wcatT = wcatT; a.whh1T = whh1T; a.h0 = h0; a.h2_all = h2_all; a.h1 = h1; a.g1 = g1;
     a.g2 = g2; a.qhp = qhp; a.alpha = alpha; a.d_h2_all = d_h2_all; a.dah = dah; a.dgi2 = dgi2; a.dqgh = dqgh; a.ds = ds;
@@ -2260,20 +2386,25 @@
     a.B = (int)B; a.Ts = (int)Ts; a.Tt = (int)Tt; a.H = (int)H; a.RT = (int)cdiv64(B, 16);
     a.pl_dq = reinterpret_cast<char*>(planes);
     a.pl_dgh1 = a.pl_dq ? a.pl_dq + Tt * a.RT * pl_block_bytes(2 * H) : nullptr;
+    a.pl_dgh2 = pl2 ? a.pl_dq + pl_base * 4 : nullptr;
+    a.pl_w2 = pl2 ? a.pl_dgh2 + Tt * a.RT * pl_block_bytes(3 * H) : nullptr;
     a.xcd_map = vag_opt().dec_xcd_map >> 4;
     VAG_TRY(sync_begin(a, sync, vag_dec_persistent_sync_words(B, Tt), s, dal, (int)(Tt * B * Ts) * ACC_SHARDS));
     int64_t lds = dec_bwd_persistent_lds_bytes(Ts, H);
     if (lds < 84 * 1024) lds = 84 * 1024;
-    if (H == 512 && !(pl ? max_lds_once<dec_bwd_persistent_kernel<64, true>>() : max_lds_once<dec_bwd_persistent_kernel<64, false>>())) return VAG_EINVAL;
-    if (H == 256 && !(pl ? max_lds_once<dec_bwd_persistent_kernel<32, true>>() : max_lds_once<dec_bwd_persistent_kernel<32, false>>())) return VAG_EINVAL;
+    const int form = pl2 ? 3 : pl ? 1 : 0;
+    bool lds_ok = false;
+    void (*kern)(DecBArgs) = nullptr;
+#define VAG_DEC_BWD_FORM(W, F) do { lds_ok = max_lds_once<dec_bwd_persistent_kernel<W, F>>(); kern = dec_bwd_persistent_kernel<W, F>; } while (0)
+    if (H == 512) { if (form == 3) VAG_DEC_BWD_FORM(64, 3); else if (form == 1) VAG_DEC_BWD_FORM(64, 1); else VAG_DEC_BWD_FORM(64, 0); }
+    else { if (form == 3) VAG_DEC_BWD_FORM(32, 3); else if (form == 1) VAG_DEC_BWD_FORM(32, 1); else VAG_DEC_BWD_FORM(32, 0); }
+#undef VAG_DEC_BWD_FORM
+    if (!lds_ok) return VAG_EINVAL;
     {
         PTimerScope timed(3, s);
         row_tile_passes(a.RT, dec_tiles_per_pass(H), [&](int rt0, int tiles) {
             a.rt0 = rt0;
-            if (H == 512 && pl) hipLaunchKernelGGL((dec_bwd_persistent_kernel<64, true>), dim3(tiles * 64u), dim3(512), (size_t)lds, s, a);
-            else if (H == 512) hipLaunchKernelGGL((dec_bwd_persistent_kernel<64, false>), dim3(tiles * 64u), dim3(512), (size_t)lds, s, a);
-            else if (pl) hipLaunchKernelGGL((dec_bwd_persistent_kernel<32, true>), dim3(tiles * 32u), dim3(512), (size_t)lds, s, a);
-            else hipLaunchKernelGGL((dec_bwd_persistent_kernel<32, false>), dim3(tiles * 32u), dim3(512), (size_t)lds, s, a);
+            hipLaunchKernelGGL(kern, dim3(tiles * (unsigned)dec_wgs(H)), dim3(512), (size_t)lds, s, a);
         });
     }
     VAG_LAUNCH_CHECK();
```

Result: faster. 22780 sentence-pairs/s, median of 6 (+1.9%).
